# evandez/neuron-descriptions

Hardware: AMD Instinct MI355X
Metric: neuron-descriptions/sec (whole node), 4096 neurons x k=15 exemplars (higher is better)
Workload: dtype f32-equivalent: operands split into (hi,lo) f16 pairs (22 significant bits), 3 f16 MFMAs per product, f32 accumulate

## Files before the change

### include/milan_hip.h

```cpp
#ifndef MILAN_HIP_H
#define MILAN_HIP_H

#include <stddef.h>
#include <stdint.h>

#ifdef __cplusplus
extern "C" {
#endif

#if defined(__GNUC__)
#pragma GCC visibility push(default)
#endif

#define MILAN_ABI_VERSION 11

enum {
  MILAN_OK = 0,
  MILAN_ERR_ARG = -1,
  MILAN_ERR_SHAPE = -2,
  MILAN_ERR_STATE = -3,
  MILAN_ERR_WORKSPACE = -4,
  MILAN_ERR_NO_LM = -5
};

// ... 18 lines not shown
  int32_t embedding_size;
  int32_t attention_size;
  int32_t vocab_size;
  int32_t start_index;
  int32_t stop_index;
  int32_t pad_index;
  int32_t has_lm;
  int32_t lm_hidden_size;
  int32_t lm_embedding_size;
  int32_t lm_layers;
  int32_t trunk_kind;
} milan_dims;

int milan_abi_version(void);
const char* milan_last_error(void);

int milan_create(milan_ctx** out, int device, const milan_dims* dims);
void milan_destroy(milan_ctx* ctx);

int milan_set_weight(milan_ctx* ctx, const char* name, const float* data,
                     const int64_t* shape, int ndim);
int milan_finalize_weights(milan_ctx* ctx, milan_stream stream);

size_t milan_workspace_bytes(const milan_ctx* ctx, int max_neurons, int k,
                             int image_size, int beam_size, int length);

int milan_encode(milan_ctx* ctx, const void* images, int image_dtype,
                 const void* masks, int mask_dtype, int n_images, int height,
                 int width, float* features, void* workspace,
                 size_t workspace_bytes, milan_stream stream);

int milan_encode_spatial(milan_ctx* ctx, const void* images, int image_dtype,
                         const void* masks, int mask_dtype, int n_images,
                         int height, int width, float* out, void* workspace,
                         size_t workspace_bytes, milan_stream stream);

int milan_init_state(milan_ctx* ctx, const float* features, int n, int k,
                     float* h, float* c, void* workspace,
                     size_t workspace_bytes, milan_stream stream);

int milan_step(milan_ctx* ctx, const float* features, int rows, int k,
               const int64_t* tokens, const float* h, const float* c,
               float* h_lm, float* c_lm, float temperature, float* predictions,
               float* attentions, float* h_out, float* c_out, void* workspace,
               size_t workspace_bytes, milan_stream stream);

int milan_decode(milan_ctx* ctx, const float* features, int n, int k,
                 int strategy, int length, int beam_size, int mi,
                 float temperature, int group_size, int64_t* tokens,
                 float* scores, float* predictions, float* attentions,
                 int64_t* beam_tokens, float* beam_scores, int32_t* out_len,
                 void* workspace, size_t workspace_bytes, milan_stream stream);

int milan_lm_score(milan_ctx* ctx, const int64_t* seqs, int rows, int L,
                   const int32_t* seq_len, float* out, void* workspace,
                   size_t workspace_bytes, milan_stream stream);

int milan_lm_logprobs(milan_ctx* ctx, const int64_t* seqs, int rows, int L,
                      float* out, void* workspace, size_t workspace_bytes,
                      milan_stream stream);

int milan_describe(milan_ctx* ctx, const void* images, int image_dtype,
                   const void* masks, int mask_dtype, int n, int k, int height,
                   int width, int strategy, int length, int beam_size, int mi,
                   float temperature, int group_size, float* features_out,
                   int64_t* tokens, float* scores, float* predictions,
                   float* attentions, int64_t* beam_tokens, float* beam_scores,
                   int32_t* out_len, void* workspace, size_t workspace_bytes,
                   milan_stream stream);

int milan_set_graph_capture(milan_ctx* ctx, int enable);
int milan_graph_stats(const milan_ctx* ctx, long long* captures,
                      long long* replays);

enum { MILAN_PRECISION_F32 = 0, MILAN_PRECISION_SPLIT_F16 = 1,
       MILAN_PRECISION_F16 = 2 };

enum { MILAN_FUSE_CHAIN = 1,
       MILAN_FUSE_CHAIN_WIDE = 2,
       MILAN_FUSE_STEM = 4,
       MILAN_FUSE_CONV3 = 8,
       MILAN_FUSE_SKIP_EMPTY = 16,
       MILAN_FUSE_BNECK = 32,
       MILAN_FUSE_SPARSE_TAIL = 64 };
int milan_set_fusion(milan_ctx* ctx, int flags);
int milan_set_precision(milan_ctx* ctx, int precision);
int milan_get_precision(const milan_ctx* ctx);

int milan_set_image_sharing(milan_ctx* ctx, int enable);
int milan_get_image_sharing(const milan_ctx* ctx);
int milan_image_sharing_stats(milan_ctx* ctx, long long* slots,
                              long long* trunk_images, int clear,
                              milan_stream stream);

enum { MILAN_STATUS_SATURATED = 1, MILAN_STATUS_NONFINITE_INPUT = 2 };
int milan_status(milan_ctx* ctx, uint32_t* flags, int clear, milan_stream stream);
int milan_set_act_scale_log2(milan_ctx* ctx, int log2_scale, milan_stream stream);
int milan_get_act_scale_log2(const milan_ctx* ctx);
int milan_encoder_absmax(milan_ctx* ctx, const void* images, int image_dtype,
                         int n_images, int height, int width, float* absmax,
                         void* workspace, size_t workspace_bytes,
                         milan_stream stream);

int milan_profile_enable(int enable);
int milan_profile_read(double* gemm_ms, double* gemm_flops,
                       long long* gemm_launches);

enum milan_stage {
  MILAN_STAGE_OTHER = 0,
  MILAN_STAGE_ENC_INPUT = 1,
  MILAN_STAGE_ENC_STEM = 2,
  MILAN_STAGE_ENC_STEM_TAIL = 3,
  MILAN_STAGE_ENC_LAYER1 = 4,
  MILAN_STAGE_ENC_LAYER2 = 5,
  MILAN_STAGE_ENC_LAYER3 = 6,
  MILAN_STAGE_ENC_LAYER4 = 7,
  MILAN_STAGE_ENC_POOL = 8,
  MILAN_STAGE_DEC_INIT = 9,
  MILAN_STAGE_DEC_SEARCH = 10,
  MILAN_STAGE_DEC_LM = 11,
  MILAN_STAGE_COUNT = 12
};
int milan_profile_read_stages(double* table );

enum milan_kernel_family {
  MILAN_KERNEL_OTHER = 0,
  MILAN_KERNEL_PP32_256 = 1,
  MILAN_KERNEL_PP32_128 = 2,
  MILAN_KERNEL_SPLIT_OTHER = 3,
  MILAN_KERNEL_F32 = 4,
  MILAN_KERNEL_CHAIN = 5,
  MILAN_KERNEL_CHAIN_WIDE = 6,
  MILAN_KERNEL_STEM = 7,
  MILAN_KERNEL_CONV3 = 8,
  MILAN_KERNEL_F16 = 9,
  MILAN_KERNEL_PP32T_256 = 10,
  MILAN_KERNEL_BNECK = 11,
  MILAN_KERNEL_COUNT = 12
};
int milan_profile_read_kernels(double* table );


int milan_exemplar_topk_update(const float* hiddens, int batch, int channels,
                               int hw, const int32_t* units, int n_units,
                               int64_t first_index, int k, int filled,
                               float* pooled_scratch, float* top_values,
                               int64_t* top_index, milan_stream stream);

int milan_exemplar_sketch_append(const float* hiddens, int batch, int channels,
                                 int hw, const int32_t* units, int n_units,
                                 int64_t first, int64_t count, float* level0,
                                 int64_t capacity, int64_t column,
                                 milan_stream stream);

size_t milan_exemplar_sort_workspace(int n_units, int64_t n, int pairs);
int milan_exemplar_sketch_compact(const float* src, int64_t src_capacity,
                                  int64_t n, int n_units, int offset, float* dst,
                                  int64_t dst_capacity, int64_t position,
                                  float* extremes, void* workspace,
                                  size_t workspace_bytes, milan_stream stream);

size_t milan_exemplar_sketch_add_workspace(int n_units, int64_t supplied,
                                           const int64_t* capacities,
                                           int n_levels);
int milan_exemplar_sketch_add(const float* hiddens, int batch, int channels, int hw,
                              const int32_t* units, int n_units, int64_t first,
                              int64_t* consumed, float* const* levels,
// ... 187 lines not shown
```

### neuron-descriptions_amd/csrc/api.hip

```cpp
#include "common.h"

#include <cstdarg>
#include <cstdio>
#include <cstring>

namespace milan {

static thread_local char g_err[1024] = "";

void set_error(const char* fmt, ...) {
  va_list ap;
  va_start(ap, fmt);
  vsnprintf(g_err, sizeof(g_err), fmt, ap);
  va_end(ap);
}

int dev_alloc(milan_ctx* c, void** p, size_t bytes) {
  if (bytes == 0) bytes = 16;
  MILAN_CHECK_HIP(hipMalloc(p, (bytes + 255) & ~size_t(255)));
  c->owned.push_back(*p);
  return 0;
}

__global__ void absmax_kernel(const float* __restrict__ w, long n,
// ... 378 lines not shown

int milan_conv2d_nhwc(const float* x, int n, int h, int w, int cin,
                      const float* weight_oihw, const float* bias, int cout,
                      int kh, int kw, int stride, int pad, int relu,
                      const float* residual, float* y, int precision,
                      milan_stream stream) {
  MILAN_REQUIRE(x && weight_oihw && y, MILAN_ERR_ARG, "conv2d: null argument");
  set_status_word(nullptr);
  const bool force_strip = precision == 3, tap_major = precision == 4, tap_linear = precision == 5;
  if (force_strip || tap_major || tap_linear) precision = MILAN_PRECISION_SPLIT_F16;
  MILAN_REQUIRE(!force_strip || MILAN_EXPERIMENTS, MILAN_ERR_ARG,
                "conv2d: the LDS-strip 3x3 kernel is only in an experiments build "
                "(make EXPERIMENTS=1)");
  MILAN_REQUIRE(precision == MILAN_PRECISION_F32 || cin % 32 == 0,
                MILAN_ERR_SHAPE, "conv2d: split-f16 needs cin %% 32 == 0");
  MILAN_REQUIRE(cin % 4 == 0 && n > 0 && cout > 0, MILAN_ERR_SHAPE,
                "conv2d: cin must be a multiple of 4");
  hipStream_t s = (hipStream_t)stream;
  const int K = kh * kw * cin, Kp = (K + 31) / 32 * 32;
  float *wp = nullptr, *zero = nullptr, *xs = nullptr, *wsp = nullptr, *ws3 = nullptr, *wst = nullptr;
  MILAN_CHECK_HIP(hipMalloc((void**)&wp, sizeof(float) * (size_t)cout * Kp));
  MILAN_CHECK_HIP(hipMalloc((void**)&zero, 256));
  MILAN_CHECK_HIP(hipMemsetAsync(zero, 0, 256, s));
  int r = pack_conv_plain(weight_oihw, cout, cin, kh, kw, wp, s);
  if (r == 0) {
    GemmArgs g{};
    const int ho = (h + 2 * pad - kh) / stride + 1, wo = (w + 2 * pad - kw) / stride + 1;
    g.A = x; g.W = wp; g.bias = bias; g.aux = residual; g.C = y;
    g.M = n * ho * wo; g.N = cout; g.K = K; g.Kp = Kp; g.ldc = cout; g.ldaux = cout;
    g.H = h; g.Wd = w; g.Cin = cin; g.Ho = ho; g.Wo = wo; g.KH = kh; g.KW = kw;
    g.stride = stride; g.pad = pad; g.a_pix_stride = cin;
    g.a_img_stride = (long)h * w * cin;
    g.epilogue = residual ? EPI_BIAS_RES_RELU : (relu ? EPI_BIAS_RELU : EPI_BIAS);
    g.zero = zero;
    if (precision == MILAN_PRECISION_SPLIT_F16) {
      const long rows = (long)n * h * w;
      hipError_t e1 = hipMalloc((void**)&xs, sizeof(float) * (size_t)rows * cin);
      hipError_t e2 = hipMalloc((void**)&wsp, sizeof(float) * (size_t)cout * Kp);
      if (e1 != hipSuccess || e2 != hipSuccess) {
        set_error("conv2d: out of memory");
        r = (int)hipErrorOutOfMemory;
      } else {
        r = launch_f32_to_split(x, cin, xs, cin, rows, cin, 1.f, s);
        if (r == 0)
          r = split_weight_into(wp, cout, Kp, wsp, &g.acc_scale,
                                reinterpret_cast<unsigned int*>(zero) + 32, s);
        g.A = xs; g.W = wsp; g.a_split = 1;
        if (r == 0 && !tap_major && kh * kw > 1 && kh * kw <= 32 && K == Kp) {
          if (hipMalloc((void**)&wst, sizeof(float) * (size_t)cout * Kp) == hipSuccess) {
            r = make_slice_major(wsp, cout, kh * kw, cin, 4, 2, wst, s);
            g.Wt = wst;
            if (tap_linear) g.tap_ncls = -1;
          }
        }
        if (MILAN_EXPERIMENTS && r == 0 && kh == 3 && kw == 3 && stride == 1 &&
            pad == 1 && K == Kp) {
          if (hipMalloc((void**)&ws3, sizeof(float) * (size_t)cout * Kp) == hipSuccess) {
            r = make_chunk_major(wsp, cout, cin, ws3, s);
            g.W3 = ws3;
            if (force_strip) g.tile_hint = 8;
          }
        }
      }
    }
    if (r == 0) r = launch_gemm(g, s);
  }
  hipError_t e = hipStreamSynchronize(s);
  (void)hipFree(wp);
  (void)hipFree(zero);
  if (xs) (void)hipFree(xs);
  if (wsp) (void)hipFree(wsp);
  if (ws3) (void)hipFree(ws3);
  if (wst) (void)hipFree(wst);
  if (r == 0 && e != hipSuccess) {
    set_error("conv2d: %s", hipGetErrorString(e));
    r = (int)e;
  }
  return r;
}

int milan_set_fusion(milan_ctx* c, int flags) {
  MILAN_REQUIRE(c, MILAN_ERR_ARG, "null ctx");
  MILAN_REQUIRE((flags & ~(MILAN_FUSE_CHAIN | MILAN_FUSE_CHAIN_WIDE | MILAN_FUSE_STEM | MILAN_FUSE_CONV3 |
                           MILAN_FUSE_SKIP_EMPTY | MILAN_FUSE_BNECK | MILAN_FUSE_SPARSE_TAIL)) == 0, MILAN_ERR_ARG,
                "unknown fusion flags %d", flags);
  c->fusion = flags;
  return 0;
}

int milan_set_image_sharing(milan_ctx* c, int enable) {
  MILAN_REQUIRE(c, MILAN_ERR_ARG, "null ctx");
  c->share_images = enable != 0;
  return 0;
}

int milan_get_image_sharing(const milan_ctx* c) { return c ? c->share_images : -1; }

int milan_image_sharing_stats(milan_ctx* c, long long* slots, long long* trunk_images, int clear,
                              milan_stream stream) {
  MILAN_REQUIRE(c && slots && trunk_images, MILAN_ERR_ARG,
                "milan_image_sharing_stats: null argument");
  hipStream_t s = (hipStream_t)stream;
  long long host[2] = {0, 0};
  MILAN_CHECK_HIP(hipMemcpyAsync(host, c->share_stats, sizeof(host), hipMemcpyDeviceToHost, s));
  if (clear) MILAN_TRY(launch_zero_fill(c->share_stats, sizeof(host), s));
  MILAN_CHECK_HIP(hipStreamSynchronize(s));
  *slots = host[0];
  *trunk_images = host[1];
  return 0;
}

int milan_set_precision(milan_ctx* c, int precision) {
  MILAN_REQUIRE(c, MILAN_ERR_ARG, "null ctx");
  MILAN_REQUIRE(precision == MILAN_PRECISION_F32 || precision == MILAN_PRECISION_SPLIT_F16 ||
                    precision == MILAN_PRECISION_F16,
                MILAN_ERR_ARG, "unknown precision mode %d", precision);
  c->trunk_f16 = precision == MILAN_PRECISION_F16;
  c->precision = c->trunk_f16 ? MILAN_PRECISION_SPLIT_F16 : precision;
  return 0;
}

int milan_get_precision(const milan_ctx* c) {
  return c ? (c->trunk_f16 ? MILAN_PRECISION_F16 : c->precision) : -1;
}

int milan_profile_enable(int enable) { return gemm_profile_enable(enable); }

int milan_profile_read(double* gemm_ms, double* gemm_flops,
                       long long* gemm_launches) {
  return gemm_profile_read(gemm_ms, gemm_flops, gemm_launches);
}

int milan_profile_read_stages(double* table) {
  MILAN_REQUIRE(table, MILAN_ERR_ARG, "milan_profile_read_stages: null table");
  return profile_read_stages(table);
}

int milan_profile_read_kernels(double* table) {
  MILAN_REQUIRE(table, MILAN_ERR_ARG, "milan_profile_read_kernels: null table");
  return profile_read_kernels(table);
}

int milan_status(milan_ctx* c, uint32_t* flags, int clear, milan_stream stream) {
  MILAN_REQUIRE(c && flags, MILAN_ERR_ARG, "milan_status: null argument");
  hipStream_t s = (hipStream_t)stream;
  unsigned host = 0;
  MILAN_CHECK_HIP(hipMemcpyAsync(&host, c->status, sizeof(host), hipMemcpyDeviceToHost, s));
  if (clear) MILAN_CHECK_HIP(hipMemsetAsync(c->status, 0, sizeof(unsigned), s));
  MILAN_CHECK_HIP(hipStreamSynchronize(s));
  *flags = host;
  return 0;
}

int milan_set_act_scale_log2(milan_ctx* c, int k, milan_stream stream) {
  MILAN_REQUIRE(c, MILAN_ERR_ARG, "null ctx");
  MILAN_REQUIRE(k >= 0 && k <= 10, MILAN_ERR_ARG,
                "activation scale 2^%d outside 2^0 .. 2^10", k);
  MILAN_REQUIRE(c->finalized, MILAN_ERR_STATE, "weights not finalized");
  c->act_scale = ldexpf(1.f, k);
  c->act_scale_log2 = k;
  return encoder_rescale(c, (hipStream_t)stream);
}

int milan_get_act_scale_log2(const milan_ctx* c) { return c ? c->act_scale_log2 : -1; }

int milan_encoder_absmax(milan_ctx* c, const void* images, int image_dtype, int n_images,
                         int height, int width, float* absmax, void* workspace,
                         size_t workspace_bytes, milan_stream stream) {
// ... 62 lines not shown
```

### neuron-descriptions_amd/csrc/common.h

```cpp
#pragma once
#include <hip/hip_runtime.h>
#include <stdint.h>
#include <stddef.h>
#include <string>
#include <vector>
#include <map>

#include "../../include/milan_hip.h"

#ifndef MILAN_EXPERIMENTS
#define MILAN_EXPERIMENTS 0
#endif

namespace milan {

void set_error(const char* fmt, ...);
#define MILAN_CHECK_HIP(expr)                                              \
  do {                                                                     \
    hipError_t _e = (expr);                                                \
    if (_e != hipSuccess) {                                                \
      milan::set_error("%s:%d: %s -> %s", __FILE__, __LINE__, #expr,       \
                       hipGetErrorString(_e));                             \
      return (int)_e;                                                      \
    }                                                                      \
  } while (0)
#define MILAN_REQUIRE(cond, code, ...)                                     \
  do {                                                                     \
    if (!(cond)) {                                                         \
      milan::set_error(__VA_ARGS__);                                       \
      return (code);                                                       \
    }                                                                      \
  } while (0)
#define MILAN_TRY(expr)                                                    \
  do {                                                                     \
    int _r = (expr);                                                       \
    if (_r != 0) return _r;                                                \
  } while (0)

enum Epilogue : int {
  EPI_BIAS = 0,
  EPI_BIAS_RELU = 1,
  EPI_BIAS_RES_RELU = 2,
  EPI_BIAS_TANH = 3,
  EPI_BIAS_SIGMUL = 4,
  EPI_BIAS_ADD = 5,
  EPI_LSTM = 6,
  EPI_LSE = 7,
};

constexpr int MILAN_TAP_CLASSES = 9;
struct GemmArgs {
  const float* A;
  const float* W;
  const float* bias;
  const float* aux;
  float* C;
  int M, N, K, Kp;
  int ldc, ldaux;
  int H, Wd, Cin, Ho, Wo, KH, KW, stride, pad;
  long a_pix_stride;
  long a_img_stride;
  int epilogue;
  const float* zero;
  int flop_k;
  int a_split;
  int out_split;
  int aux_split;
  float acc_scale;
  int out_mode;
  const float* W3;
  const float* A2;
  int K1, H2, W2d, stride2;
  long a2_pix_stride, a2_img_stride;
  int aniso, stride_w, pad_w;
  int debug;
  int tile_hint;
  int stagger;
  long long* prof;
  int chunk_major;
  float* C2;
  float* Cs;
  unsigned* status;
  int f16;
  const float* Wt;
  int tap_inner;
  const long long* lse_tgt;
  long lse_tgt_stride;
  float* lse_x;
  const int* m_live;
  int m_live_mul;
  int tap_ncls;
  int tap_cls[MILAN_TAP_CLASSES][5];
};
static_assert(sizeof(GemmArgs) % 4 == 0, "GemmArgs is reloaded word by word");

enum OutMode : int { OUT_SCALAR = 0, OUT_VEC4 = 1, OUT_SPLIT8 = 2, OUT_F16 = 3 };

int launch_gemm(const GemmArgs& g, hipStream_t s);
void set_status_word(unsigned* word);
unsigned* status_word();
void profile_tag_kernel(int family);
int launch_zero_fill(void* p, size_t bytes, hipStream_t s);
int launch_f32_to_split(const float* src, long ld_src, float* dst, long ld_dst,
                        long rows, int K, float scale, hipStream_t s);
int gemm_profile_enable(int enable);
int ensure_lds_attr(const void* kern, int bytes);
int device_cus8(int* out);
void* gemm_profile_begin(double flops, double bytes, hipStream_t s);
void gemm_profile_end(void* rec, hipStream_t s);

struct ShareArgs {
  const unsigned char* images;
  long bytes;
  int n;
  int hash_bits;
  int skip_empty;
  const int* list_n;
  const int* bbox;
  void* hash;
  int *rep, *flag;
  int *order, *bbox_c, *count, *class_of;
};
int launch_image_classes(const ShareArgs& a, hipStream_t s);
int launch_share_count(long long* stats, int n, const int* live, hipStream_t s);

struct ChainArgs {
  const float* T2;
  const float* W3;
  const float* bias3;
  const float* R;
  float* X;
  const float* W1;
  const float* bias1;
  float* T1;
  int M, P;
  const float* A2;
  int KD;
  float scale3, scale1;
  long long* prof;
  int NR;
  unsigned* status;
  const int* m_live;
  int m_live_mul;
  const float* C2in;
  const float* W2;
  const float* bias2;
  float scale2;
  int ch, cw;
  const float* W0;
  const float* bias0;
  float scale0;
};
bool chain_supported(int P, int KD, int NR = 0);
bool chain_conv_supported(int P, int KD, int NR, int h, int w);
bool chain_conv_c1_supported(int P, int KD, int NR, int h, int w);
int launch_chain(const ChainArgs& a, hipStream_t s);
struct StemArgs {
  const float* in;
  const float* ws;
  const float* bias;
  float acc_scale;
  const float* scale;
  const float* shift;
  float* raw;
  float* y;
  const int* bbox;
  const float* zero;
  int n, H, G, h1, w1, hp, wp;
  int tiles_y, tiles_x;
  int debug;
  unsigned* status;
  const unsigned char* in_u8;
  const unsigned* lut;
  const int* order;
  int W;
  const int* n_live;
};
bool stem_fused_supported(int cout, int Kp);
int launch_stem_fused(const StemArgs& a, hipStream_t s);
struct Conv3Args {
  const float* in;
// ... 119 lines not shown

__device__ __forceinline__ float cvt_pk_f16(float a, float b) {
  float r;
  asm("v_cvt_pk_f16_f32 %0, %1, %2" : "=v"(r) : "v"(a), "v"(b));
  return r;
}
template <int SEL>
__device__ __forceinline__ float mix_sub_f16(float x, float hpair) {
  float r;
  if constexpr (SEL == 0)
    asm("v_fma_mix_f32 %0, -%1, 1.0, %2 op_sel:[0,0,0] op_sel_hi:[1,0,0]" : "=v"(r) : "v"(hpair), "v"(x));
  else
    asm("v_fma_mix_f32 %0, -%1, 1.0, %2 op_sel:[1,0,0] op_sel_hi:[1,0,0]" : "=v"(r) : "v"(hpair), "v"(x));
  return r;
}
template <int SEL>
__device__ __forceinline__ float mix_add_f16(float hpair, float lpair) {
  float r;
  if constexpr (SEL == 0)
    asm("v_fma_mix_f32 %0, %1, 1.0, %2 op_sel:[0,0,0] op_sel_hi:[1,0,1]" : "=v"(r) : "v"(hpair), "v"(lpair));
  else
    asm("v_fma_mix_f32 %0, %1, 1.0, %2 op_sel:[1,0,1] op_sel_hi:[1,0,1]" : "=v"(r) : "v"(hpair), "v"(lpair));
  return r;
}
__device__ __forceinline__ float max3_abs(float a, float b, float c) {
  float r;
  asm("v_max3_f32 %0, |%1|, |%2|, |%3|" : "=v"(r) : "v"(a), "v"(b), "v"(c));
  return r;
}
__device__ __forceinline__ float sat_fold8(const float* x, float sat) {
  return max3_abs(max3_abs(x[0], x[1], x[2]), max3_abs(x[3], x[4], x[5]), max3_abs(x[6], x[7], sat));
}
__device__ __forceinline__ void report_saturation(unsigned* status, float sat) {
  if (status != nullptr && sat >= 65504.f) atomicOr(status, 1u );
}
template <typename V4>
__device__ __forceinline__ void split8_rne(const float* v, V4* hi_out, V4* lo_out, float* sat = nullptr) {
  V4 hi, lo;
  float x[8];
#pragma unroll
  for (int d = 0; d < 4; ++d) {
    asm("v_med3_f32 %0, %1, %2, %3" : "=v"(x[2 * d]) : "v"(v[2 * d]), "v"(-65504.f), "v"(65504.f));
    asm("v_med3_f32 %0, %1, %2, %3" : "=v"(x[2 * d + 1]) : "v"(v[2 * d + 1]), "v"(-65504.f), "v"(65504.f));
    hi[d] = cvt_pk_f16(x[2 * d], x[2 * d + 1]);
    lo[d] = cvt_pk_f16(mix_sub_f16<0>(x[2 * d], hi[d]), mix_sub_f16<1>(x[2 * d + 1], hi[d]));
  }
  if (sat) *sat = sat_fold8(x, *sat);
  *hi_out = hi;
  *lo_out = lo;
}
template <typename V4>
__device__ __forceinline__ void split8_relu_rne(const float* v, V4* hi_out, V4* lo_out, float* sat = nullptr) {
  V4 hi, lo;
  float x[8];
#pragma unroll
  for (int d = 0; d < 4; ++d) {
    asm("v_med3_f32 %0, %1, 0, %2" : "=v"(x[2 * d]) : "v"(v[2 * d]), "v"(65504.f));
    asm("v_med3_f32 %0, %1, 0, %2" : "=v"(x[2 * d + 1]) : "v"(v[2 * d + 1]), "v"(65504.f));
    hi[d] = cvt_pk_f16(x[2 * d], x[2 * d + 1]);
    lo[d] = cvt_pk_f16(mix_sub_f16<0>(x[2 * d], hi[d]), mix_sub_f16<1>(x[2 * d + 1], hi[d]));
  }
  if (sat) *sat = sat_fold8(x, *sat);
  *hi_out = hi;
  *lo_out = lo;
}
template <typename V4>
__device__ __forceinline__ void join8_exact(V4 hi, V4 lo, float* v) {
#pragma unroll
  for (int d = 0; d < 4; ++d) {
    v[2 * d] = mix_add_f16<0>(hi[d], lo[d]);
    v[2 * d + 1] = mix_add_f16<1>(hi[d], lo[d]);
  }
}

}

struct milan_ctx {
  int device = 0;
  milan_dims d{};
  bool finalized = false;
  int precision = 0;
  int trunk_f16 = 0;
  int fusion = MILAN_FUSE_CHAIN | MILAN_FUSE_CHAIN_WIDE | MILAN_FUSE_STEM | MILAN_FUSE_CONV3 |
               MILAN_FUSE_SKIP_EMPTY | MILAN_FUSE_BNECK | MILAN_FUSE_SPARSE_TAIL;
  int graph_capture = 0;
  struct GraphEntry { std::vector<char> key; hipGraphExec_t exec = nullptr; int seen = 0; };
  std::vector<GraphEntry> graphs;
  long graph_replays = 0, graph_captures = 0;
  float* scratch = nullptr;
  size_t scratch_floats = 0;
  std::map<std::string, milan::Tensor> raw;
  std::vector<void*> owned;
  float* zero = nullptr;
  milan::ConvW stem;
  milan::ConvW stem_pair;
  milan::ConvW alex[5];
  float *bn1_scale = nullptr, *bn1_shift = nullptr;
  float act_scale = 32.f;
  int act_scale_log2 = 5;
  float *bn1_scale_s = nullptr, *bn1_shift_s = nullptr;
  unsigned* stem_lut = nullptr;
  unsigned* status = nullptr;
  unsigned* calib = nullptr;
  int share_images = 0;
  int share_hash_bits = 64;
  long long* share_stats = nullptr;
  std::vector<milan::Bottleneck> blocks[4];
  float mean[3] = {0.485f, 0.456f, 0.406f}, stdv[3] = {0.229f, 0.224f, 0.225f};
  milan::LinearW init_h, init_c, q2h, k2h, gate, lstm_ih, lstm_hh, out;
  milan::LinearW lstm_cat;
  float *att_w = nullptr, *att_b = nullptr;
  float* embedding = nullptr;
  std::vector<milan::LinearW> lm_ih, lm_hh;
  std::vector<milan::LinearW> lm_cat;
  milan::LinearW lm_out;
  float* lm_embedding = nullptr;
};

namespace milan {
int dev_alloc(milan_ctx* c, void** p, size_t bytes);
int make_split_weight(milan_ctx* c, const float* w, int n, int kp, float** ws,
                      float* ws_inv, hipStream_t s);
int pack_conv_plain(const float* w_oihw, int cout, int cin, int kh, int kw,
                    float* wp, hipStream_t s);
int encoder_finalize(milan_ctx* c, hipStream_t s);
int encoder_rescale(milan_ctx* c, hipStream_t s);
int make_slice_major(const float* ws, int cout, int taps, int cin, int gps, int gb, float* dst,
                     hipStream_t s);
int make_chunk_major(const float* ws, int cout, int cin, float* dst,
                     hipStream_t s);
size_t encoder_workspace(const milan_ctx* c, int n_images, int H, int W);
int encoder_run_spatial(milan_ctx* c, const void* images, int image_dtype,
                        const void* masks, int mask_dtype, int n, int H, int W,
                        float* out, milan::Arena& ws, hipStream_t s);
int encoder_run(milan_ctx* c, const void* images, int image_dtype,
                const void* masks, int mask_dtype, int n_images, int H, int W,
                float* features, Arena& ws, hipStream_t s);
int decoder_finalize(milan_ctx* c, hipStream_t s);
size_t decoder_workspace(const milan_ctx* c, int n, int k, int beam, int length);
int decoder_init_state(milan_ctx* c, const float* features, int n, int k,
                       float* h, float* cc, Arena& ws, hipStream_t s);
int decoder_step(milan_ctx* c, const float* features, int rows, int k,
                 const int64_t* tokens, const float* h, const float* cc,
                 float* h_lm, float* c_lm, float temperature,
                 float* predictions, float* attentions, float* h_out,
                 float* c_out, Arena& ws, hipStream_t s);
int decoder_decode(milan_ctx* c, const float* features, int n, int k,
                   int strategy, int length, int beam, int mi,
                   float temperature, int group_size, int64_t* tokens,
                   float* scores, float* predictions, float* attentions,
                   int64_t* beam_tokens, float* beam_scores, int32_t* out_len,
                   Arena& ws, hipStream_t s);
int decoder_lm_logprobs(milan_ctx* c, const int64_t* seqs, int rows, int L,
                        float* out, milan::Arena& ws, hipStream_t s);
int decoder_lm_score(milan_ctx* c, const int64_t* seqs, int rows, int L,
                     const int32_t* seq_len, float* out, Arena& ws,
                     hipStream_t s);
}
```

### neuron-descriptions_amd/csrc/encoder.hip

```cpp
#include "common.h"
#include <optional>
#include <vector>

#include <cstdlib>

namespace milan {

static constexpr float kBnEps = 1e-5f;

__global__ void pack_conv_kernel(const float* __restrict__ w, int cout, int cin,
                                 int cinp, int kh, int kw, int kp,
                                 const float* __restrict__ gamma,
                                 const float* __restrict__ beta,
                                 const float* __restrict__ mean,
                                 const float* __restrict__ var,
                                 float* __restrict__ wp,
                                 float* __restrict__ bias) {
  const long total = (long)cout * kp;
  for (long idx = blockIdx.x * (long)blockDim.x + threadIdx.x; idx < total;
       idx += (long)gridDim.x * blockDim.x) {
    const int o = idx / kp, k = idx - (long)o * kp;
    const int tap = k / cinp, i = k - tap * cinp;
    float v = 0.f;
    if (tap < kh * kw && i < cin) {
// ... 769 lines not shown
  if constexpr (SHARED) {
    img = blockIdx.x;
    const int cls = class_of[img];
    if (cls < img0 || cls >= img0 + ncls) return;
    trow = cls - img0;
  } else {
    const int slot_img = blockIdx.x + img0;
    if (live != nullptr && slot_img >= *live) return;
    img = order ? order[slot_img] : slot_img;
    trow = blockIdx.x;
  }
  const int lane = threadIdx.x & 63, wave = threadIdx.x >> 6;
  const int G = C / 8, pw = 64 / lpp;
  const int gl = lane % lpp, sub = lane / lpp;
  const int g = blockIdx.y * 64 + gl;
  const int slot = wave * pw + sub, nslots = 4 * pw;
  const long base = (long)img * lv.per_image + lv.off[level];
  const int cnt = list_n[img * 5 + level];
  const float* t = tap + (long)trow * P * C + (long)g * 8;
  float a0[8], a1[8];
#pragma unroll
  for (int e = 0; e < 8; ++e) { a0[e] = 0.f; a1[e] = 0.f; }
  auto add = [&](int i, float (&acc)[8]) {
    const float* q = t + (long)list_idx[base + i] * C;
    const float w = list_w[base + i];
    const f32x4_t hi = *reinterpret_cast<const f32x4_t*>(q);
    const f32x4_t lo = *reinterpret_cast<const f32x4_t*>(q + 4);
    float v[8];
    join8_exact(hi, lo, v);
#pragma unroll
    for (int e = 0; e < 8; ++e) acc[e] += w * v[e];
  };
  if (g < G) {
    int i = slot;
    for (; i + nslots < cnt; i += 2 * nslots) { add(i, a0); add(i + nslots, a1); }
    if (i < cnt) add(i, a0);
  }
#pragma unroll
  for (int e = 0; e < 8; ++e) part[(wave * 64 + lane) * 8 + e] = a0[e] + a1[e];
  __syncthreads();
  if (wave == 0 && sub == 0 && g < G) {
    float sum[8];
#pragma unroll
    for (int e = 0; e < 8; ++e) sum[e] = 0.f;
    for (int w = 0; w < 4; ++w)
      for (int sb = 0; sb < pw; ++sb)
#pragma unroll
        for (int e = 0; e < 8; ++e) sum[e] += part[(w * 64 + sb * lpp + gl) * 8 + e];
    const bool bad = poison != nullptr && poison[img];
    float* f = features + (long)img * fstride + col_off + g * 8;
#pragma unroll
    for (int e = 0; e < 8; ++e) f[e] = bad ? __builtin_nanf("") : sum[e] * inv_scale;
  }
}

__global__ void poison_fill_kernel(float* __restrict__ out, long per_image, int n,
                                   const int* __restrict__ poison) {
  const long total = (long)n * per_image;
  for (long i = blockIdx.x * (long)blockDim.x + threadIdx.x; i < total;
       i += (long)gridDim.x * blockDim.x)
    if (poison[i / per_image]) out[i] = __builtin_nanf("");
}

__global__ void act_absmax_kernel(const float* __restrict__ x, long n,
                                  unsigned* __restrict__ out) {
  float m = 0.f;
  for (long i = blockIdx.x * (long)blockDim.x + threadIdx.x; i < n;
       i += (long)gridDim.x * blockDim.x) {
    const float a = fabsf(x[i]);
    m = (a > m || a != a) ? a : m;
  }
  for (int o = 32; o > 0; o >>= 1) {
    const float t = __shfl_xor(m, o);
    m = (t > m || t != t) ? t : m;
  }
  if ((threadIdx.x & 63) == 0) atomicMax(out, __float_as_uint(m));
}


constexpr int kTailMaxP = 1024;

__global__ __launch_bounds__(64) void tail_union_kernel(
    const int* __restrict__ list_idx, const int* __restrict__ list_n, Levels lv,
    const int* __restrict__ class_of, int P, unsigned char* __restrict__ s0) {
  const int i = blockIdx.x, c = class_of[i];
  if (c < 0) return;
  const long base = (long)i * lv.per_image + lv.off[4];
  const int cnt = list_n[i * 5 + 4];
  for (int e = threadIdx.x; e < cnt; e += 64) s0[(long)c * P + list_idx[base + e]] = 1;
}

__global__ __launch_bounds__(64) void tail_sets_kernel(
    const int* __restrict__ list_idx, const int* __restrict__ list_n, Levels lv,
    const int* __restrict__ order, const int* __restrict__ live, int n,
    int* __restrict__ loc, int* __restrict__ cnt,
    const unsigned char* __restrict__ s0 = nullptr) {
  __shared__ unsigned char s[3][kTailMaxP];
  const int j = blockIdx.x, lane = threadIdx.x;
  const int h = lv.h[4], w = lv.w[4], P = h * w;
  if (live != nullptr && j >= *live) {
    if (lane < 3) cnt[lane * n + j] = 0;
    return;
  }
  const int img = order ? order[j] : j;
  if (s0 != nullptr) {
    for (int p = lane; p < P; p += 64) s[0][p] = s0[(long)j * P + p];
  } else {
    for (int p = lane; p < P; p += 64) s[0][p] = 0;
    __syncthreads();
    const long base = (long)img * lv.per_image + lv.off[4];
    const int c = list_n[img * 5 + 4];
    for (int i = lane; i < c; i += 64) s[0][list_idx[base + i]] = 1;
  }
  __syncthreads();
  for (int k = 1; k < 3; ++k) {
    for (int p = lane; p < P; p += 64) {
      const int y = p / w, x = p - y * w;
      unsigned char v = 0;
      for (int dy = -1; dy <= 1; ++dy)
        for (int dx = -1; dx <= 1; ++dx) {
          const int yy = y + dy, xx = x + dx;
          if (yy >= 0 && yy < h && xx >= 0 && xx < w) v |= s[k - 1][yy * w + xx];
        }
      s[k][p] = v;
    }
    __syncthreads();
  }
  for (int k = 0; k < 3; ++k) {
    int count = 0;
    int* out = loc + ((long)k * n + j) * P;
    for (int p0 = 0; p0 < P; p0 += 64) {
      const int p = p0 + lane;
      const bool nz = p < P && s[k][p];
      const unsigned long long m = __ballot(nz);
      if (nz) out[count + __popcll(m & ((1ull << lane) - 1ull))] = p;
      count += __popcll(m);
    }
    if (lane == 0) cnt[k * n + j] = count;
  }
}

__global__ __launch_bounds__(256) void tail_scan_kernel(const int* __restrict__ cnt, int n,
                                                        int* __restrict__ off, int* __restrict__ U) {
  __shared__ int tmp[256];
  const int k = blockIdx.x, tid = threadIdx.x;
  int base = 0;
  for (int j0 = 0; j0 < n; j0 += 256) {
    const int j = j0 + tid;
    const int v = j < n ? cnt[(long)k * n + j] : 0;
    tmp[tid] = v;
    __syncthreads();
    for (int o = 1; o < 256; o <<= 1) {
      const int add = tid >= o ? tmp[tid - o] : 0;
      __syncthreads();
      tmp[tid] += add;
      __syncthreads();
    }
    if (j < n) off[(long)k * n + j] = base + tmp[tid] - v;
    base += tmp[255];
    __syncthreads();
  }
  if (tid == 0) U[k] = base;
}

__global__ void tail_fill_kernel(const int* __restrict__ loc, const int* __restrict__ cnt,
                                 const int* __restrict__ off, int n, int P, int* __restrict__ rows) {
  const int j = blockIdx.x, k = blockIdx.y;
  const int c = cnt[k * n + j], o = off[k * n + j];
  for (int i = threadIdx.x; i < c; i += blockDim.x)
    rows[(long)k * n * P + o + i] = j * P + loc[((long)k * n + j) * P + i];
}

template <bool SCATTER>
__global__ void tail_rows_kernel(const float4* __restrict__ src, const int* __restrict__ idx,
                                 const int* __restrict__ live, int w4, float4* __restrict__ dst) {
  const long total = (long)*live * w4;
  for (long i = blockIdx.x * (long)blockDim.x + threadIdx.x; i < total;
       i += (long)gridDim.x * blockDim.x) {
    const long u = i / w4;
    const int q = (int)(i - u * w4);
    if (SCATTER) dst[(long)idx[u] * w4 + q] = src[i];
    else dst[i] = src[(long)idx[u] * w4 + q];
  }
}

__global__ void tail_im2col_kernel(const float4* __restrict__ t1, const int* __restrict__ rows,
                                   const int* __restrict__ live, int h, int w, int C,
                                   float4* __restrict__ acol) {
  const int per = 9 * C / 4, P = h * w, c4 = C / 4;
  const long total = (long)*live * per;
  for (long i = blockIdx.x * (long)blockDim.x + threadIdx.x; i < total;
       i += (long)gridDim.x * blockDim.x) {
    const long u = i / per;
    const int q = (int)(i - u * per);
    const int sl = q / 72, r = q - sl * 72, tap = r >> 3, f = r & 7;
    const int row = rows[u];
    const int j = row / P, p = row - j * P;
    const int y = p / w + tap / 3 - 1, x = p % w + tap % 3 - 1;
    float4 v = make_float4(0.f, 0.f, 0.f, 0.f);
    if (y >= 0 && y < h && x >= 0 && x < w)
      v = t1[((long)j * P + y * w + x) * c4 + sl * 8 + f];
    acol[i] = v;
  }
}

struct EncPlan {
  Levels lv;
  int h1, w1, hp, wp;
  float *in4, *raw, *x0, *x1, *ds, *t1, *t2;
  size_t x_sz, t1_sz, t2_sz;
  int *list_idx, *list_n;
  float* list_w;
  int* bbox;
  int* poison;
  int *order, *bbox_c, *count;
  int *tail_loc, *tail_cnt, *tail_off, *tail_rows, *tail_U;
  void* sh_hash;
  int *sh_rep, *sh_flag, *class_of;
  unsigned char* tail_s0;
};

static int conv_out(int h, int k, int s, int p) { return (h + 2 * p - k) / s + 1; }

static int plan(const milan_ctx* c, int n, int H, int W, Arena& a, EncPlan* pl) {
  const int wd = c->d.trunk_width;
  pl->h1 = conv_out(H, 7, 2, 3); pl->w1 = conv_out(W, 7, 2, 3);
  pl->hp = conv_out(pl->h1, 3, 2, 1); pl->wp = conv_out(pl->w1, 3, 2, 1);
  Levels& lv = pl->lv;
  lv.h[0] = pl->h1; lv.w[0] = pl->w1;
  lv.h[1] = pl->hp; lv.w[1] = pl->wp;
  for (int l = 2; l < 5; ++l) {
    lv.h[l] = conv_out(lv.h[l - 1], 3, 2, 1);
    lv.w[l] = conv_out(lv.w[l - 1], 3, 2, 1);
  }
  long off = 0;
  for (int l = 0; l < 5; ++l) { lv.off[l] = off; off += (long)lv.h[l] * lv.w[l]; }
  lv.per_image = off;
  const int exp = c->d.trunk_kind == MILAN_TRUNK_BASIC ? 1 : 4;
  size_t x_sz = (size_t)pl->hp * pl->wp * wd, t1_sz = 0, t2_sz = 0;
  for (int li = 0; li < 4; ++li) {
    const size_t planes = (size_t)wd << li;
    const size_t in_px = (size_t)lv.h[li == 0 ? 1 : li] * lv.w[li == 0 ? 1 : li];
    const size_t out_px = (size_t)lv.h[li + 1] * lv.w[li + 1];
    x_sz = x_sz > out_px * planes * exp ? x_sz : out_px * planes * exp;
    t1_sz = t1_sz > in_px * planes ? t1_sz : in_px * planes;
    t2_sz = t2_sz > out_px * planes ? t2_sz : out_px * planes;
  }
  pl->x_sz = x_sz; pl->t1_sz = t1_sz; pl->t2_sz = t2_sz;
  pl->in4 = a.get<float>((size_t)n * H * (W + 2) * 4);
  pl->raw = a.get<float>((size_t)n * pl->h1 * pl->w1 * wd);
  pl->x0 = a.get<float>((size_t)n * x_sz);
  pl->x1 = a.get<float>((size_t)n * x_sz);
  pl->ds = a.get<float>((size_t)n * x_sz);
  pl->t1 = a.get<float>((size_t)n * t1_sz);
  pl->t2 = a.get<float>((size_t)n * t2_sz);
  pl->list_idx = a.get<int>((size_t)n * lv.per_image);
  pl->list_w = a.get<float>((size_t)n * lv.per_image);
  pl->list_n = a.get<int>((size_t)n * 5);
  pl->bbox = a.get<int>((size_t)n * 4);
  pl->poison = a.get<int>((size_t)n);
  pl->order = a.get<int>((size_t)n);
  pl->bbox_c = a.get<int>((size_t)n * 4);
  pl->count = a.get<int>(4);
  {
    const size_t P4 = (size_t)lv.h[4] * lv.w[4];
    pl->tail_loc = a.get<int>(3 * (size_t)n * P4);
    pl->tail_rows = a.get<int>(3 * (size_t)n * P4);
    pl->tail_cnt = a.get<int>(3 * (size_t)n);
    pl->tail_off = a.get<int>(3 * (size_t)n);
    pl->tail_U = a.get<int>(4);
    pl->sh_hash = a.get<unsigned long long>((size_t)n);
    pl->sh_rep = a.get<int>((size_t)n);
    pl->sh_flag = a.get<int>((size_t)n);
    pl->class_of = a.get<int>((size_t)n);
    pl->tail_s0 = a.get<unsigned char>(((size_t)n * P4 + 3) & ~(size_t)3);
  }
  return 0;
}

static int encoder_sub_batch() {
  static int v = 0;
  if (v == 0) {
    const char* e = getenv("MILAN_ENC_SUB");
    v = e ? atoi(e) : 9600;
    if (v < 1) v = 9600;
  }
  return v;
}

static void alexnet_workspace_dry(const milan_ctx* c, int n, int H, int W,
                                  Arena& a);

size_t encoder_workspace(const milan_ctx* c, int n_images, int H, int W) {
  Arena a; a.dry = true;
  const int sub = encoder_sub_batch();
  const int n = n_images < sub ? n_images : sub;
  if (c->d.trunk_kind == MILAN_TRUNK_NONE) return 0;
  if (c->d.trunk_kind == MILAN_TRUNK_ALEXNET) {
    alexnet_workspace_dry(c, n, H, W, a);
    return a.off;
  }
  EncPlan pl;
  plan(c, n, H, W, a, &pl);
  return a.off;
}

static GemmArgs conv_args(const ConvW& cw, const float* in, int n, int H, int W,
                          float* out, int epi, const float* aux,
                          const float* zero, int* Ho, int* Wo,
                          bool split = false, bool scaled_bias = true) {
  GemmArgs g{};
  *Ho = conv_out(H, cw.kh, cw.stride, cw.pad);
  *Wo = conv_out(W, cw.kw, cw.stride, cw.pad);
  g.A = in; g.W = cw.w; g.bias = cw.bias; g.aux = aux; g.C = out;
  g.M = n * (*Ho) * (*Wo); g.N = cw.cout; g.K = cw.K; g.Kp = cw.Kp;
  g.ldc = cw.cout; g.ldaux = cw.cout;
  g.H = H; g.Wd = W; g.Cin = cw.cin; g.Ho = *Ho; g.Wo = *Wo;
  g.KH = cw.kh; g.KW = cw.kw; g.stride = cw.stride; g.pad = cw.pad;
  g.a_pix_stride = cw.cin;
  g.a_img_stride = (long)H * W * cw.cin;
  g.epilogue = epi; g.zero = zero;
  g.flop_k = cw.kh * cw.kw * cw.cin_real;
  if (split) {
    g.W = cw.ws; g.a_split = 1; g.out_split = 1; g.aux_split = aux != nullptr;
    g.acc_scale = cw.ws_inv;
    g.W3 = cw.ws3;
    g.Wt = cw.wst;
    if (scaled_bias && cw.bias_s) g.bias = cw.bias_s;
  }
  return g;
}

static GemmArgs conv_args_f16(const ConvW& cw, const float* in, int n, int H, int W,
                              float* out, int epi, const float* aux, const float* zero,
                              int* Ho, int* Wo) {
  GemmArgs g = conv_args(cw, in, n, H, W, out, epi, aux, zero, Ho, Wo, true);
  g.W = cw.wf; g.W3 = nullptr; g.Wt = cw.wft;
  g.f16 = 1; g.out_split = 0; g.aux_split = 0;
  g.Cin = cw.cin / 2; g.K = cw.K / 2; g.Kp = cw.Kp / 2;
  g.a_pix_stride = cw.cin / 2;
  g.a_img_stride = (long)H * W * (cw.cin / 2);
  g.ldc = cw.cout / 2; g.ldaux = cw.cout / 2;
  return g;
}

static int encoder_run_batch(milan_ctx* c, const void* images, int image_dtype,
                             const void* masks, int mask_dtype, int n, int H,
                             int W, float* features, Arena& ws, hipStream_t s,
                             float* spatial_out = nullptr);
static int alexnet_run_batch(milan_ctx* c, const void* images, int image_dtype,
                             const void* masks, int mask_dtype, int n, int H,
                             int W, float* features, Arena& ws, hipStream_t s);

int encoder_run(milan_ctx* c, const void* images, int image_dtype,
                const void* masks, int mask_dtype, int n, int H, int W,
                float* features, Arena& ws, hipStream_t s) {
  const int sub = encoder_sub_batch();
  const size_t isz = image_dtype == MILAN_DTYPE_U8 ? 1 : 4;
// ... 227 lines not shown
    else
      hipLaunchKernelGGL(masked_pool_kernel<0>, dim3(cnt, (C + 63) / 64),
                         dim3(256), 0, s, tap, P, C, level, pl.lv, pl.list_idx,
                         pl.list_w, pl.list_n, features, F, col_off, img0, 1.f, poison, order, live);
    MILAN_CHECK_HIP(hipGetLastError());
    return 0;
  };

  int ho, wo;
  {
    GemmArgs g = conv_args(c->stem, pl.in4, n, H, W, pl.raw, EPI_BIAS, nullptr,
                           c->zero, &ho, &wo);
    if (pair_stem) {
      g = conv_args(c->stem_pair, pl.in4, n, H, G, pl.raw, EPI_BIAS, nullptr,
                    c->zero, &ho, &wo, true);
      g.Ho = ho = pl.h1; g.Wo = wo = pl.w1;
      g.M = n * ho * wo;
      g.aniso = 1; g.stride_w = 1; g.pad_w = 1;
      g.out_split = 0;
      g.flop_k = c->stem.kh * c->stem.kw * c->stem.cin_real;
    }
    const bool fused_stem = pair_stem && (c->fusion & MILAN_FUSE_STEM) &&
                            stem_fused_supported(c->stem_pair.cout, c->stem_pair.Kp);
    if (fused_stem) {
      StemArgs sa{};
      sa.in = pl.in4; sa.ws = c->stem_pair.ws; sa.bias = c->stem_pair.bias;
      if (stem_u8) {
        sa.in = nullptr; sa.in_u8 = (const unsigned char*)images; sa.lut = c->stem_lut;
        sa.order = order; sa.W = W;
      }
      sa.n_live = live;
      sa.acc_scale = c->stem_pair.ws_inv;
      sa.scale = c->bn1_scale_s; sa.shift = c->bn1_shift_s;
      sa.raw = spatial ? nullptr : pl.raw; sa.y = pl.x0;
      sa.bbox = spatial ? nullptr : bbox;
      sa.zero = c->zero;
      sa.n = n; sa.H = H; sa.G = G; sa.h1 = pl.h1; sa.w1 = pl.w1;
      sa.hp = pl.hp; sa.wp = pl.wp;
      {
        StageScope scope(MILAN_STAGE_ENC_STEM, s);
        MILAN_TRY(launch_stem_fused(sa, s));
      }
      MILAN_TRY(pool(pl.raw, 0, wd, 0));
    } else {
    {
      StageScope scope(MILAN_STAGE_ENC_STEM, s);
      MILAN_TRY(launch_live(g));
    }
    MILAN_TRY(pool(pl.raw, 0, wd, 0));
    stage.emplace(MILAN_STAGE_ENC_STEM_TAIL, s);
    const long total = (long)n * pl.hp * pl.wp * (wd / (split ? 8 : 4));
    const int blocks = (int)((total + 255) / 256 < 16384 ? (total + 255) / 256 : 16384);
    if (split)
      hipLaunchKernelGGL(bn_relu_maxpool_split_kernel, dim3(blocks), dim3(256), 0,
                         s, pl.raw, n, pl.h1, pl.w1, wd, pl.hp, pl.wp,
                         c->bn1_scale_s, c->bn1_shift_s, pl.x0, c->status, live);
    else
      hipLaunchKernelGGL(bn_relu_maxpool_kernel, dim3(blocks), dim3(256), 0, s,
                         (const float4*)pl.raw, n, pl.h1, pl.w1, wd / 4, pl.hp,
                         pl.wp, (const float4*)c->bn1_scale,
                         (const float4*)c->bn1_shift, (float4*)pl.x0, live);
    MILAN_CHECK_HIP(hipGetLastError());
    stage.reset();
    }
    if (c->calib && !split) {
      MILAN_TRY(track(pl.x0, (long)n * pl.hp * pl.wp * wd));
    }
  }

  auto gemm_t = [&](const GemmArgs& g) -> int {
    MILAN_TRY(launch_live(g));
    if (c->calib && !split) MILAN_TRY(track(g.C, (long)g.M * g.N));
    return 0;
  };
  const int P4 = pl.lv.h[4] * pl.lv.w[4];
  bool tail = split && !fast && !spatial && masks != nullptr && c->calib == nullptr &&
              (c->fusion & MILAN_FUSE_SPARSE_TAIL) && c->d.trunk_kind == MILAN_TRUNK_BOTTLENECK &&
              c->blocks[3].size() >= 2 && P4 >= 1 && P4 <= kTailMaxP;
  if (tail) {
    const Bottleneck& lb = c->blocks[3].back();
    const size_t need = (size_t)P4 * ((size_t)2 * lb.c1.cin + lb.c3.cout + (size_t)11 * lb.c1.cout);
    tail = need <= (size_t)pl.h1 * pl.w1 * wd;
  }
  if (tail) {
    const unsigned char* s0 = nullptr;
    if (class_of != nullptr) {
      MILAN_TRY(launch_zero_fill(pl.tail_s0, ((size_t)n * P4 + 3) & ~(size_t)3, s));
      hipLaunchKernelGGL(tail_union_kernel, dim3(n), dim3(64), 0, s, pl.list_idx, pl.list_n, pl.lv,
                         class_of, P4, pl.tail_s0);
      s0 = pl.tail_s0;
    }
    hipLaunchKernelGGL(tail_sets_kernel, dim3(n), dim3(64), 0, s, pl.list_idx, pl.list_n, pl.lv,
                       order, live, n, pl.tail_loc, pl.tail_cnt, s0);
    hipLaunchKernelGGL(tail_scan_kernel, dim3(3), dim3(256), 0, s, pl.tail_cnt, n, pl.tail_off,
                       pl.tail_U);
    hipLaunchKernelGGL(tail_fill_kernel, dim3(n, 3), dim3(64), 0, s, pl.tail_loc, pl.tail_cnt,
                       pl.tail_off, n, P4, pl.tail_rows);
    MILAN_CHECK_HIP(hipGetLastError());
  }
  auto tail_block_ok = [&](const Bottleneck& b) {
    return !b.basic && !b.has_down && b.c1.ws && b.c2.ws && b.c2.wst && b.c3.ws && b.c1.bias_s &&
           b.c2.bias_s && b.c3.bias_s && b.c1.kh == 1 && b.c1.kw == 1 && b.c1.stride == 1 &&
           b.c2.kh == 3 && b.c2.kw == 3 && b.c2.stride == 1 && b.c2.pad == 1 && b.c3.kh == 1 &&
           b.c3.kw == 1 && b.c3.stride == 1 && b.c1.K == b.c1.Kp && b.c2.K == b.c2.Kp &&
           b.c3.K == b.c3.Kp && b.c1.cout % 32 == 0 && b.c2.cin == b.c1.cout &&
           b.c2.cout == b.c1.cout && b.c3.cin == b.c1.cout && b.c3.cout == b.c1.cin &&
           b.c1.cin % 4 == 0;
  };
  auto tail_block = [&](const Bottleneck& b, const float* X, float* Y, float* T1, int hh,
                        int ww, int kM, int kO) -> int {
    const long rows_all = (long)n * P4;
    const int Cin = b.c1.cin, P = b.c1.cout, Cout = b.c3.cout;
    float* xg = pl.raw;
    float* t1c = xg + rows_all * Cin;
    float* acol = t1c + rows_all * P;
    float* t2c = acol + rows_all * 9 * P;
    float* rg = t2c + rows_all * P;
    float* yc = rg + rows_all * Cin;
    const int* rowsM = pl.tail_rows + (long)kM * n * P4;
    const int* rowsO = pl.tail_rows + (long)kO * n * P4;
    const int* UM = pl.tail_U + kM;
    const int* UO = pl.tail_U + kO;
    auto blocks_for = [](long items) { return (int)((items + 255) / 256 < 8192 ? (items + 255) / 256 : 8192); };
    auto lin = [&](const float* A, int K, const ConvW& cw, const float* W, float* C, int N, int epi,
                   const float* aux, const int* U) -> int {
      GemmArgs g = linear_args(A, K, W, cw.bias_s, C, N, (int)rows_all, N, K, epi, c->zero, aux, N);
      g.a_split = 1; g.out_split = 1; g.aux_split = aux != nullptr;
      g.acc_scale = cw.ws_inv;
      g.flop_k = cw.kh * cw.kw * cw.cin_real;
      g.m_live = U; g.m_live_mul = 1;
      return launch_gemm(g, s);
    };
    hipLaunchKernelGGL(tail_rows_kernel<false>, dim3(blocks_for(rows_all * (Cin / 4))), dim3(256), 0, s,
                       (const float4*)X, rowsM, UM, Cin / 4, (float4*)xg);
    MILAN_TRY(lin(xg, Cin, b.c1, b.c1.ws, t1c, P, EPI_BIAS_RELU, nullptr, UM));
    hipLaunchKernelGGL(tail_rows_kernel<true>, dim3(blocks_for(rows_all * (P / 4))), dim3(256), 0, s,
                       (const float4*)t1c, rowsM, UM, P / 4, (float4*)T1);
    hipLaunchKernelGGL(tail_im2col_kernel, dim3(blocks_for(rows_all * (9 * P / 4))), dim3(256), 0, s,
                       (const float4*)T1, rowsO, UO, hh, ww, P, (float4*)acol);
    MILAN_TRY(lin(acol, 9 * P, b.c2, b.c2.wst, t2c, P, EPI_BIAS_RELU, nullptr, UO));
    hipLaunchKernelGGL(tail_rows_kernel<false>, dim3(blocks_for(rows_all * (Cin / 4))), dim3(256), 0, s,
                       (const float4*)X, rowsO, UO, Cin / 4, (float4*)rg);
    MILAN_TRY(lin(t2c, P, b.c3, b.c3.ws, yc, Cout, EPI_BIAS_RES_RELU, rg, UO));
    hipLaunchKernelGGL(tail_rows_kernel<true>, dim3(blocks_for(rows_all * (Cout / 4))), dim3(256), 0, s,
                       (const float4*)yc, rowsO, UO, Cout / 4, (float4*)Y);
    MILAN_CHECK_HIP(hipGetLastError());
    return 0;
  };

  float *x = pl.x0, *y = pl.x1;
  int h = pl.hp, w = pl.wp, col = wd;
  bool t1_ready = false;
  float *t1buf = pl.t1, *t1alt = pl.ds;
  for (int li = 0; li < 4; ++li) {
    stage.emplace(MILAN_STAGE_ENC_LAYER1 + li, s);
    const std::vector<Bottleneck>& blocks = c->blocks[li];
    if (fast && li == 2) {
      const long groups = (long)n * h * w * ((wd * 4) << 1) / 8;
      const int nb = (int)((groups + 255) / 256 < 16384 ? (groups + 255) / 256 : 16384);
      hipLaunchKernelGGL(split_to_f16_kernel, dim3(nb), dim3(256), 0, s, x, groups, pl.ds, live,
                         groups / n);
      MILAN_CHECK_HIP(hipGetLastError());
      y = x; x = pl.ds;
    }
    for (size_t bi = 0; bi < blocks.size(); ++bi) {
      const Bottleneck& b = blocks[bi];
      int h1, w1, h2, w2, h3, w3;
      if (fast && li >= 2) {
        GemmArgs g1 = conv_args_f16(b.c1, x, n, h, w, pl.t1, EPI_BIAS_RELU, nullptr, c->zero, &h1, &w1);
        MILAN_TRY(launch_live(g1));
        GemmArgs g2 = conv_args_f16(b.c2, pl.t1, n, h1, w1, pl.t2, EPI_BIAS_RELU, nullptr, c->zero, &h2, &w2);
        MILAN_TRY(launch_live(g2));
        if (b.has_down) {
          GemmArgs g3 = conv_args_f16(b.c3d, pl.t2, n, h2, w2, y, EPI_BIAS_RELU, nullptr, c->zero, &h3, &w3);
          g3.Cin = b.c3.cin / 2;
          g3.a_pix_stride = b.c3.cin / 2;
          g3.a_img_stride = (long)h2 * w2 * (b.c3.cin / 2);
          g3.A2 = x; g3.K1 = b.c3.K / 2; g3.H2 = h; g3.W2d = w;
          g3.stride2 = b.down.stride;
          g3.a2_pix_stride = b.down.cin / 2;
          g3.a2_img_stride = (long)h * w * (b.down.cin / 2);
          g3.flop_k = b.c3.K + b.down.K;
          MILAN_TRY(launch_live(g3));
        } else {
          GemmArgs g3 = conv_args_f16(b.c3, pl.t2, n, h2, w2, y, EPI_BIAS_RES_RELU, x, c->zero, &h3, &w3);
          MILAN_TRY(launch_live(g3));
        }
        float* tmp = x; x = y; y = tmp;
        h = h3; w = w3;
        continue;
      }
      if (tail && li == 3 && bi >= 1 && bi + 2 >= blocks.size() && tail_block_ok(b) &&
          (bi + 1 == blocks.size() || tail_block_ok(blocks.back())) &&
          h == pl.lv.h[4] && w == pl.lv.w[4]) {
        const int kO = bi + 1 == blocks.size() ? 0 : 1;
        MILAN_TRY(tail_block(b, x, y, t1buf, h, w, kO + 1, kO));
        float* tmp = x; x = y; y = tmp;
        continue;
      }
      if (b.basic) {
        GemmArgs g1 = conv_args(b.c1, x, n, h, w, pl.t1, EPI_BIAS_RELU, nullptr,
                                c->zero, &h1, &w1, split);
        MILAN_TRY(gemm_t(g1));
        const float* identity = x;
        if (b.has_down) {
          int hd, wdn;
          GemmArgs gd = conv_args(b.down, x, n, h, w, pl.ds, EPI_BIAS, nullptr,
                                  c->zero, &hd, &wdn, split);
          MILAN_TRY(gemm_t(gd));
          identity = pl.ds;
        }
        GemmArgs g2 = conv_args(b.c2, pl.t1, n, h1, w1, y, EPI_BIAS_RES_RELU,
                                identity, c->zero, &h3, &w3, split);
        MILAN_TRY(gemm_t(g2));
        float* tmp = x; x = y; y = tmp;
        h = h3; w = w3;
        continue;
      }
      GemmArgs g1 = conv_args(b.c1, x, n, h, w, t1buf, EPI_BIAS_RELU, nullptr,
                              c->zero, &h1, &w1, split);
      const bool c1_pending = !t1_ready;
      t1_ready = false;
      GemmArgs g2 = conv_args(b.c2, t1buf, n, h1, w1, pl.t2, EPI_BIAS_RELU,
                              nullptr, c->zero, &h2, &w2, split);
#if MILAN_EXPERIMENTS
      {
        static const bool taps_inner = getenv("MILAN_TAPS_INNER") && atoi(getenv("MILAN_TAPS_INNER"));
        if (split && taps_inner && b.c2.ws3 && b.c2.cin >= 128 && b.c2.cout > 64) {
          g2.W = b.c2.ws3;
          g2.chunk_major = 1;
          g2.W3 = nullptr;
        }
      }
#endif
      const bool last_of_stage = bi + 1 == blocks.size();
      const Bottleneck* nbp = !last_of_stage ? &blocks[bi + 1]
                              : (li + 1 < 4 && !c->blocks[li + 1].empty())
                                    ? &c->blocks[li + 1][0] : nullptr;
      bool chain_plain = false, chain_ds = false;
      int chain_P = 0, chain_NR = 0;
      if (split && nbp != nullptr && !(fast && last_of_stage && li + 1 >= 2) && !b.basic &&
          (c->fusion & (b.c3.cin >= 256 ? MILAN_FUSE_CHAIN_WIDE : MILAN_FUSE_CHAIN))) {
        const Bottleneck& nb = *nbp;
        chain_P = b.c3.cin;
        chain_NR = last_of_stage ? 2 * chain_P : chain_P;
        const bool shapes = !nb.basic && nb.has_down == last_of_stage && nb.c1.ws &&
                            b.c3.ws && b.c3.kh == 1 && b.c3.kw == 1 && b.c3.stride == 1 &&
                            b.c3.K == b.c3.Kp && b.c3.cout == 4 * chain_P &&
                            nb.c1.kh == 1 && nb.c1.kw == 1 && nb.c1.stride == 1 &&
                            nb.c1.cin == 4 * chain_P && nb.c1.cout == chain_NR &&
                            nb.c1.K == nb.c1.Kp && b.c3.bias && nb.c1.bias;
        h2 = conv_out(h1, b.c2.kh, b.c2.stride, b.c2.pad);
        w2 = conv_out(w1, b.c2.kw, b.c2.stride, b.c2.pad);
        chain_plain = shapes && !b.has_down && chain_supported(chain_P, 0, chain_NR);
        chain_ds = shapes && b.has_down && b.c3d.ws && b.down.kh == 1 &&
                   b.down.kw == 1 && b.down.stride == 1 && h2 == h &&
                   w2 == w && chain_supported(chain_P, b.down.cin, chain_NR);
      }
      const bool conv_front =
          (chain_plain || chain_ds) && (c->fusion & MILAN_FUSE_BNECK) && b.c2.K == b.c2.Kp &&
          b.c2.bias_s && conv3_p64_supported(b.c2.cin, b.c2.cout, b.c2.kh, b.c2.kw, b.c2.stride,
                                             b.c2.pad) &&
          chain_conv_supported(chain_P, chain_ds ? b.down.cin : 0, chain_NR, h1, w1);
      const bool c1_front =
          conv_front && c1_pending && chain_ds && b.c1.ws && b.c1.bias_s && b.c1.kh == 1 &&
          b.c1.kw == 1 && b.c1.stride == 1 && b.c1.cin == 64 && b.c1.cout == 64 &&
          b.c1.K == b.c1.Kp && h1 == h && w1 == w &&
          chain_conv_c1_supported(chain_P, b.down.cin, chain_NR, h1, w1);
      if (c1_pending && !c1_front) MILAN_TRY(gemm_t(g1));
      if (conv_front) {
      } else if (split && (c->fusion & MILAN_FUSE_CONV3) && b.c2.K == b.c2.Kp &&
          conv3_p64_supported(b.c2.cin, b.c2.cout, b.c2.kh, b.c2.kw, b.c2.stride,
                              b.c2.pad)) {
        Conv3Args ca{};
        ca.in = t1buf; ca.ws = b.c2.ws; ca.bias = b.c2.bias_s; ca.acc_scale = b.c2.ws_inv;
        ca.out = pl.t2; ca.zero = c->zero; ca.n = n; ca.h = h1; ca.w = w1;
        ca.n_live = live;
        MILAN_TRY(launch_conv3_p64(ca, s));
      } else {
        MILAN_TRY(gemm_t(g2));
      }
      const float* identity = x;
      if (chain_plain || chain_ds) {
        const Bottleneck& nb = *nbp;
        ChainArgs ca{};
        ca.T2 = pl.t2; ca.X = y; ca.W1 = nb.c1.ws; ca.bias1 = nb.c1.bias_s;
        ca.T1 = t1buf; ca.M = n * h2 * w2; ca.P = chain_P; ca.scale1 = nb.c1.ws_inv;
        ca.NR = chain_NR;
        ca.m_live = live; ca.m_live_mul = h2 * w2;
        if (conv_front) {
          ca.C2in = t1buf; ca.W2 = b.c2.ws; ca.bias2 = b.c2.bias_s; ca.scale2 = b.c2.ws_inv;
          ca.ch = h1; ca.cw = w1;
          ca.T2 = nullptr; ca.T1 = t1alt;
          if (c1_front) {
            ca.C2in = x; ca.W0 = b.c1.ws; ca.bias0 = b.c1.bias_s; ca.scale0 = b.c1.ws_inv;
          }
        }
        if (chain_plain) {
          ca.W3 = b.c3.ws; ca.bias3 = b.c3.bias_s; ca.R = x; ca.scale3 = b.c3.ws_inv;
        } else {
          ca.W3 = b.c3d.ws; ca.bias3 = b.c3d.bias_s; ca.A2 = x; ca.KD = b.down.cin;
          ca.scale3 = b.c3d.ws_inv;
        }
        MILAN_TRY(launch_chain(ca, s));
        if (conv_front) { float* tt = t1buf; t1buf = t1alt; t1alt = tt; }
        t1_ready = true;
        float* tmp = x; x = y; y = tmp;
        h = h2; w = w2;
        continue;
      }
      if (b.has_down && split && b.c3d.ws && b.c3d.cout > 64) {
        int h3, w3;
        GemmArgs g3 = conv_args(b.c3d, pl.t2, n, h2, w2, y, EPI_BIAS_RELU,
                                nullptr, c->zero, &h3, &w3, true);
        g3.Cin = b.c3.cin;
        g3.a_pix_stride = b.c3.cin;
        g3.a_img_stride = (long)h2 * w2 * b.c3.cin;
        g3.A2 = x; g3.K1 = b.c3.K; g3.H2 = h; g3.W2d = w;
        g3.stride2 = b.down.stride;
        g3.a2_pix_stride = b.down.cin;
        g3.a2_img_stride = (long)h * w * b.down.cin;
        g3.flop_k = b.c3.K + b.down.K;
        MILAN_TRY(gemm_t(g3));
        float* tmp = x; x = y; y = tmp;
        h = h3; w = w3;
        continue;
      }
      if (b.has_down) {
        int hd, wdn;
        GemmArgs gd = conv_args(b.down, x, n, h, w, pl.ds, EPI_BIAS, nullptr,
                                c->zero, &hd, &wdn, split);
        MILAN_TRY(gemm_t(gd));
        identity = pl.ds;
      }
      GemmArgs g3 = conv_args(b.c3, pl.t2, n, h2, w2, y, EPI_BIAS_RES_RELU,
                              identity, c->zero, &h3, &w3, split);
      MILAN_TRY(gemm_t(g3));
      float* tmp = x; x = y; y = tmp;
      h = h3; w = w3;
    }
    stage.reset();
    const int C = (c->d.trunk_kind == MILAN_TRUNK_BASIC ? wd : wd * 4) << li;
    MILAN_REQUIRE(h == pl.lv.h[li + 1] && w == pl.lv.w[li + 1], MILAN_ERR_SHAPE,
                  "internal: stage %d geometry mismatch", li + 1);
    MILAN_TRY(pool(x, li + 1, C, col));
    col += C;
  }
  if (spatial) {
    const int C = (c->d.trunk_kind == MILAN_TRUNK_BASIC ? wd : wd * 4) << 3;
    const long rows = (long)n * h * w;
    if (split) {
      const long total = rows * (C / 8);
      const int blocks = (int)((total + 255) / 256 < 16384 ? (total + 255) / 256 : 16384);
      hipLaunchKernelGGL(split_to_f32_kernel, dim3(blocks), dim3(256), 0, s, x,
                         total, spatial_out, 1.f / c->act_scale);
      MILAN_CHECK_HIP(hipGetLastError());
    } else {
      MILAN_CHECK_HIP(hipMemcpyAsync(spatial_out, x, sizeof(float) * rows * C,
                                     hipMemcpyDeviceToDevice, s));
    }
    if (poison) {
      const long per_image = (long)h * w * C;
      const long total = (long)n * per_image;
      const int blocks = (int)((total + 255) / 256 < 4096 ? (total + 255) / 256 : 4096);
      hipLaunchKernelGGL(poison_fill_kernel, dim3(blocks), dim3(256), 0, s, spatial_out,
                         per_image, n, poison);
      MILAN_CHECK_HIP(hipGetLastError());
    }
  }
  return 0;
}

int encoder_rescale(milan_ctx* c, hipStream_t s) {
  auto redo = [&](const float* src, float* dst, int n) -> int {
    if (!src || !dst) return 0;
    hipLaunchKernelGGL(scale_vec_kernel, dim3((n + 255) / 256), dim3(256), 0, s, src,
                       c->act_scale, n, dst);
    MILAN_CHECK_HIP(hipGetLastError());
    return 0;
  };
  if (c->stem.w) {
    MILAN_TRY(redo(c->bn1_scale, c->bn1_scale_s, c->stem.cout));
    MILAN_TRY(redo(c->bn1_shift, c->bn1_shift_s, c->stem.cout));
  }
  for (int li = 0; li < 4; ++li)
    for (Bottleneck& b : c->blocks[li])
      for (ConvW* w : {&b.c1, &b.c2, &b.c3, &b.down, &b.c3d})
        MILAN_TRY(redo(w->bias, w->bias_s, w->cout));
  return 0;
}


__global__ void maxpool3s2_f32_kernel(const float4* __restrict__ x, int n, int H,
                                      int W, int C4, int Ho, int Wo, int pad,
                                      float4* __restrict__ y) {
  const long total = (long)n * Ho * Wo * C4;
  for (long idx = blockIdx.x * (long)blockDim.x + threadIdx.x; idx < total;
       idx += (long)gridDim.x * blockDim.x) {
    const int cc = idx % C4;
    long t = idx / C4;
    const int wo = t % Wo; t /= Wo;
    const int ho = t % Ho;
    const long img = t / Ho;
    float4 best = make_float4(-INFINITY, -INFINITY, -INFINITY, -INFINITY);
    for (int dy = 0; dy < 3; ++dy) {
// ... 204 lines not shown
```

### neuron-descriptions_amd/csrc/gemm.hip

```cpp
#include "common.h"

#include <map>
#include <mutex>
#include <utility>

#include <cstdio>
#include <cstdlib>
#include <cstring>
#include <type_traits>
#include <utility>
#include <vector>

#ifndef MILAN_ABLATE_BUILD
#define MILAN_ABLATE_BUILD 0
#endif
#ifndef MILAN_EXPERIMENTS
#define MILAN_EXPERIMENTS 0
#endif

namespace milan {

typedef float f32x16 __attribute__((ext_vector_type(16)));
typedef float f32x4 __attribute__((ext_vector_type(4)));
typedef _Float16 f16x8 __attribute__((ext_vector_type(8)));
// ... 1117 lines not shown
        for (int it = 0; it < B_ITERS; ++it) issue_b(it, kt_issue, nxt_slot);
        __builtin_amdgcn_sched_barrier(0);
      }
#pragma unroll
      for (int i = 0; i < TM; ++i) {
        if (i + 1 < TM) {
          ah[i + 1] = *reinterpret_cast<const f32x4*>(Ab + aoff[i + 1] +
                                                      ((chi ^ aswz[i + 1]) << 2));
          al[i + 1] = *reinterpret_cast<const f32x4*>(Ab + aoff[i + 1] +
                                                      ((clo ^ aswz[i + 1]) << 2));
        }
        if constexpr (STEADY) {
          if constexpr (DMA_POS == 0) {
            if (i < A_ITERS) issue_a(ra, i, kt_issue, nxt_slot);
            else issue_b(i - A_ITERS, kt_issue, nxt_slot);
          }
        } else {
          if (i < A_ITERS && has_next) issue_a(ra_n, i, kt_issue, nxt_slot);
        }
#pragma unroll
        for (int j = 0; j < TN; ++j) {
          acc[i][j] = __builtin_amdgcn_mfma_f32_32x32x16_f16(
              as_f16x8(ah[i]), as_f16x8(bl[j]), acc[i][j], 0, 0, 0);
          acc[i][j] = __builtin_amdgcn_mfma_f32_32x32x16_f16(
              as_f16x8(al[i]), as_f16x8(bh[j]), acc[i][j], 0, 0, 0);
          acc[i][j] = __builtin_amdgcn_mfma_f32_32x32x16_f16(
              as_f16x8(ah[i]), as_f16x8(bh[j]), acc[i][j], 0, 0, 0);
        }
      }
      if constexpr (STEADY && DMA_POS == 2) {
        __builtin_amdgcn_sched_barrier(0);
#pragma unroll
        for (int it = 0; it < A_ITERS; ++it) issue_a(ra, it, kt_issue, nxt_slot);
#pragma unroll
        for (int it = 0; it < B_ITERS; ++it) issue_b(it, kt_issue, nxt_slot);
      }
    };
    auto advance = [&]() { cur = cur + 1 == STAGES ? 0 : cur + 1; };
    auto slot_ahead = [&]() { const int n = cur + AHEAD; return n >= STAGES ? n - STAGES : n; };

    auto steady_loop = [&](auto pos_tag) {
      for (int kt = 0; kt + AHEAD < nk; ++kt) {
        compute(cur, slot_ahead(), kt + AHEAD, std::true_type{}, pos_tag);
        asm volatile("s_waitcnt vmcnt(%0)" ::"n"((AHEAD - 1) * LOADS) : "memory");
        __builtin_amdgcn_s_barrier();
        advance();
      }
    };
    if (wave < NT_WAVES / 2) steady_loop(std::integral_constant<int, 1>{});
    else steady_loop(std::integral_constant<int, 2>{});
#pragma unroll
    for (int t = 0; t < AHEAD; ++t) {
      compute(cur, slot_ahead(), t, std::false_type{}, std::integral_constant<int, 0>{});
      if (t + 1 < AHEAD) {
        if (has_next) {
          if (t == 0) asm volatile("s_waitcnt vmcnt(%0)" ::"n"(2 * LOADS + A_ITERS) : "memory");
          else if (t == 1) asm volatile("s_waitcnt vmcnt(%0)" ::"n"(LOADS + 2 * A_ITERS) : "memory");
          else asm volatile("s_waitcnt vmcnt(%0)" ::"n"(3 * A_ITERS) : "memory");
        } else {
          if (t == 0) asm volatile("s_waitcnt vmcnt(%0)" ::"n"(2 * LOADS) : "memory");
          else if (t == 1) asm volatile("s_waitcnt vmcnt(%0)" ::"n"(LOADS) : "memory");
          else asm volatile("s_waitcnt vmcnt(0)" ::: "memory");
        }
        __builtin_amdgcn_s_barrier();
      }
      advance();
    }
    __builtin_amdgcn_s_barrier();
#pragma unroll
    for (int i = 0; i < TM; ++i)
#pragma unroll
      for (int j = 0; j < TN; ++j) acc[i][j] = acc[i][j] * g.acc_scale;
    run_epilogue<TM, TN>(g, acc, Bs, wave, lane, tile_m * BM + wm * WROWS,
                         tile_n * BN + wn * 64);
    if (!has_next) break;
    __builtin_amdgcn_s_barrier();
    q += gridDim.x;
    tile_m = ntile_m; tile_n = ntile_n;
#pragma unroll
    for (int it = 0; it < A_ITERS; ++it) ra[it] = ra_n[it];
  }
}

__device__ __forceinline__ GemmArgs reload_gemm_args() {
  typedef const int __attribute__((address_space(4)))* KArgWords;
  KArgWords kw = (KArgWords)__builtin_amdgcn_kernarg_segment_ptr();
  asm volatile("" : "+s"(kw));
  GemmArgs g;
  int words[sizeof(GemmArgs) / 4];
#pragma unroll
  for (unsigned i = 0; i < sizeof(GemmArgs) / 4; ++i) words[i] = kw[i];
  __builtin_memcpy(&g, words, sizeof(GemmArgs));
  g.M = live_rows(g.m_live, g.m_live_mul, g.M);
  return g;
}


__device__ __forceinline__ void split16_pp_tile(int tile_m, int tile_n, int tid) {
  const GemmArgs g = reload_gemm_args();
  constexpr int BM = 256, BN = 256, BK = 16, S = 4, TM = 4, TN = 2, LOADS = 4;
  constexpr unsigned OOB = 0x80000000u;
  extern __shared__ __attribute__((aligned(16))) float smem[];
  float* As = smem;
  float* Bs = smem + S * BM * BK;
  const int lane = tid & 63;
  const int wave = __builtin_amdgcn_readfirstlane(tid >> 6);
  const int wm = wave >> 2, wn = wave & 3;

  const int lrow = tid >> 2;
  const int kc = (tid & 3) ^ ((tid >> 4) & 3);
  const int HoWo = g.Ho * g.Wo;
  const int img0 = (tile_m * BM) / HoWo;
  const long bias = ((long)g.pad * g.Wd + g.pad) * g.a_pix_stride;
  const __amdgpu_buffer_rsrc_t srd_a = __builtin_amdgcn_make_buffer_rsrc(
      const_cast<float*>(g.A + (long)img0 * g.a_img_stride - bias), 0, 0x7fffffff, 0x00020000);
  const __amdgpu_buffer_rsrc_t srd_a2 = __builtin_amdgcn_make_buffer_rsrc(
      const_cast<float*>(g.A2 ? g.A2 + (long)img0 * g.a2_img_stride : g.A), 0, 0x7fffffff,
      0x00020000);
  const __amdgpu_buffer_rsrc_t srd_w = __builtin_amdgcn_make_buffer_rsrc(
      const_cast<float*>(g.W + (long)tile_n * BN * g.Kp), 0, 0x7fffffff, 0x00020000);
  unsigned row_off[2], row_off2[2], voff[2], vb[2];
  int hi0[2], wi0[2];
#pragma unroll
  for (int it = 0; it < 2; ++it) {
    const int m = tile_m * BM + it * 128 + lrow;
    const bool ok = m < g.M;
    const int mm = ok ? m : g.M - 1;
    const int img = mm / HoWo;
    const int rem = mm - img * HoWo;
    const int ho = rem / g.Wo, wo = rem - ho * g.Wo;
    hi0[it] = ho * g.stride - g.pad;
    wi0[it] = wo * g.stride - g.pad;
    row_off[it] = ok ? (unsigned)(((long)(img - img0) * g.a_img_stride +
                                   ((long)hi0[it] * g.Wd + wi0[it]) * g.a_pix_stride + bias +
                                   kc * 4) * 4)
                     : OOB;
    row_off2[it] = (ok && g.A2)
                       ? (unsigned)(((long)(img - img0) * g.a2_img_stride +
                                     ((long)(ho * g.stride2) * g.W2d + wo * g.stride2) *
                                         g.a2_pix_stride + kc * 4) * 4)
                       : OOB;
    const int n = tile_n * BN + it * 128 + lrow;
    vb[it] = n < g.N ? (unsigned)(((long)(it * 128 + lrow) * g.Kp + kc * 4) * 4) : OOB;
  }
  const int nk = g.Kp / BK;
  const int k1_tiles = g.A2 ? g.K1 / BK : 0x7fffffff;
  int is_kt = 0, is_kh = 0, is_kw = 0, is_cin0 = 0, seg_soff = 0;
  int cin_limit = g.Cin;
  __amdgpu_buffer_rsrc_t cur_srd = srd_a;
  auto set_tap = [&]() {
#pragma unroll
    for (int it = 0; it < 2; ++it) {
      const bool inb = (unsigned)(hi0[it] + is_kh) < (unsigned)g.H &&
                       (unsigned)(wi0[it] + is_kw) < (unsigned)g.Wd;
      voff[it] = inb ? row_off[it] : OOB;
    }
    seg_soff = (int)((((long)is_kh * g.Wd + is_kw) * g.a_pix_stride) * 4);
  };
  set_tap();
  auto issue_tile = [&](auto slot_tag) {
    constexpr int SLOT = decltype(slot_tag)::value;
    int woff = wave * (16 * BK);
    asm volatile("" : "+s"(woff));
    float* adst = As + SLOT * (BM * BK) + woff;
    float* bdst = Bs + SLOT * (BN * BK) + woff;
    const int soff = seg_soff + is_cin0 * 4;
    __builtin_amdgcn_raw_ptr_buffer_load_lds(cur_srd, (LDS_AS void*)adst, 16, voff[0], soff, 0, 0);
    __builtin_amdgcn_raw_ptr_buffer_load_lds(cur_srd, (LDS_AS void*)(adst + 128 * BK), 16, voff[1],
                                             soff, 0, 0);
    const int woffk = is_kt * (BK * 4);
    __builtin_amdgcn_raw_ptr_buffer_load_lds(srd_w, (LDS_AS void*)bdst, 16, vb[0], woffk, 0, 0);
    __builtin_amdgcn_raw_ptr_buffer_load_lds(srd_w, (LDS_AS void*)(bdst + 128 * BK), 16, vb[1],
                                             woffk, 0, 0);
    if (is_kt + 1 < nk) {
      ++is_kt;
      is_cin0 += BK;
// ... 103 lines not shown
  } else {
    phase_barrier();
    auto step = [&](auto slot_tag) {
      read_phase(slot_tag);
      asm volatile("s_waitcnt vmcnt(%0)" ::"n"((S - 2) * LOADS) : "memory");
      phase_barrier();
      multiply();
      phase_barrier();
    };
    int kt = 0;
    for (; kt + 4 <= nk; kt += 4) {
      step(std::integral_constant<int, 0>{});
      step(std::integral_constant<int, 1>{});
      step(std::integral_constant<int, 2>{});
      step(std::integral_constant<int, 3>{});
    }
    if (kt < nk) {
      step(std::integral_constant<int, 0>{});
      step(std::integral_constant<int, 1>{});
    }
  }
  asm volatile("s_waitcnt vmcnt(0)" ::: "memory");
  __builtin_amdgcn_s_barrier();
  const GemmArgs ge = reload_gemm_args();
#pragma unroll
  for (int i = 0; i < TM; ++i)
#pragma unroll
    for (int j = 0; j < TN; ++j) acc[i][j] = acc[i][j] * ge.acc_scale;
  run_epilogue<TM, TN>(ge, acc, smem, wave, lane, tile_m * BM + wm * 128, tile_n * BN + wn * 64);
}

struct PpLoader {
  __amdgpu_buffer_rsrc_t srd_a, srd_a2, srd_w, cur_srd;
  unsigned row_off[4], row_off2[4], voff[4], vb[4];
  int hw0[4];
  unsigned mask[4];
  int ia, iw, is_kh, is_kw, is_cin0, seg_soff, cin_limit;
  unsigned a_bits, w_bits;
  int w_slice;
};

struct TapTile {
  int y0, ny, x0, nx;
  unsigned mask;
  int cnt, j, tile_n;
};

__device__ __forceinline__ bool tap_tile(const GemmArgs& g, int tiles_m, int tiles_n, TapTile* t) {
  const int b = blockIdx.x;
  if (g.tap_ncls == 0) {
    const int T = tiles_m * tiles_n;
    if (b >= T) return false;
    const int tile = xcd_tile(b, T);
    t->j = tile / tiles_n;
    t->tile_n = tile - t->j * tiles_n;
    t->y0 = 0; t->ny = g.Ho; t->x0 = 0; t->nx = g.Wo;
    t->mask = 0xffffffffu >> (32 - g.KH * g.KW);
    t->cnt = g.M;
    return true;
  }
  typedef const int __attribute__((address_space(4)))* KArgWords;
  const KArgWords cw = (KArgWords)__builtin_amdgcn_kernarg_segment_ptr() + offsetof(GemmArgs, tap_cls) / 4;
  const int imgs = g.M / (g.Ho * g.Wo);
  int first = 0, cls = -1, cfirst = 0, ctiles = 0;
#pragma unroll
  for (int c = 0; c < MILAN_TAP_CLASSES; ++c) {
    const int T = c < g.tap_ncls ? ((imgs * cw[c * 5 + 1] * cw[c * 5 + 3] + 255) >> 8) * tiles_n : 0;
    const int B = (T + 7) & ~7;
    if (cls < 0 && b < first + B) { cls = c; cfirst = first; ctiles = T; }
    first += B;
  }
  if (cls < 0) return false;
  const int bl = b - cfirst;
  if ((bl >> 3) >= (ctiles >> 3) + ((bl & 7) < (ctiles & 7))) return false;
  const int tile = xcd_tile(bl, ctiles);
  t->j = tile / tiles_n;
  t->tile_n = tile - t->j * tiles_n;
  t->y0 = cw[cls * 5]; t->ny = cw[cls * 5 + 1]; t->x0 = cw[cls * 5 + 2]; t->nx = cw[cls * 5 + 3];
  t->mask = (unsigned)cw[cls * 5 + 4];
  t->cnt = imgs * t->ny * t->nx;
  return true;
}

template <int BNW, bool F16 = false, bool TAPI = false>
__device__ __forceinline__ void split16_pp32_tile(int tile_m, int tile_n, int tid, bool prefetched,
                                                  bool has_next, int ntile_m, int ntile_n,
                                                  TapTile tt = TapTile{}) {
  const GemmArgs g = reload_gemm_args();
  constexpr int BM = 256, BN = 256, BKP = 32, TM = BNW == 256 ? 4 : 2, TN = 2;
  static_assert(BNW == 256 || BNW == 128, "ping-pong tile: 256 or 128 columns");
  constexpr int SLOTF = BM * BKP;
  constexpr unsigned OOB = 0x80000000u;
  extern __shared__ __attribute__((aligned(16))) float smem[];
  auto a_slot = [&](int sl) { return smem + (sl < 2 ? sl : 3) * SLOTF; };
  auto w_slot = [&](int sl) { return smem + (sl == 0 ? 2 : 4) * SLOTF; };
  const int lane = tid & 63;
  const int wave = __builtin_amdgcn_readfirstlane(tid >> 6);
  const int wm = BNW == 256 ? wave >> 2 : wave >> 1, wn = BNW == 256 ? wave & 3 : wave & 1;
  const int group = wave >> 2;
  const int HoWo = g.Ho * g.Wo;
  const int np = TAPI ? (g.Cin / BKP) * __builtin_popcount(tt.mask) : g.Kp / BKP;
  const int k1_pairs = g.A2 ? g.K1 / BKP : 0x7fffffff;
  const int KHKW = g.KH * g.KW;
  const int r_kw = 65536 / g.KW + 1;

  auto set_tap = [&](PpLoader& L) {
    if constexpr (TAPI) {
      const int t = __builtin_ctz(L.a_bits);
      const int kh = (t * r_kw) >> 16, kw = t - kh * g.KW;
#pragma unroll
      for (int it = 0; it < 4; ++it) L.voff[it] = (L.mask[it] >> t) & 1u ? L.row_off[it] : OOB;
      L.seg_soff = (int)((((long)kh * g.Wd + kw) * g.a_pix_stride) * 4);
      return;
    }
#pragma unroll
    for (int it = 0; it < 4; ++it) {
      const int hi = (L.hw0[it] >> 16) + L.is_kh, wi = (int)(short)(L.hw0[it] & 0xffff) + L.is_kw;
      const bool inb = (unsigned)hi < (unsigned)g.H && (unsigned)wi < (unsigned)g.Wd;
      L.voff[it] = inb ? L.row_off[it] : OOB;
    }
    L.seg_soff = (int)((((long)L.is_kh * g.Wd + L.is_kw) * g.a_pix_stride) * 4);
  };
  const int pix_img = TAPI ? tt.ny * tt.nx : HoWo, pix_row = TAPI ? tt.nx : g.Wo;
  const int rows_all = TAPI ? tt.cnt : g.M;
  const float r_howo = 1.0f / (float)pix_img, r_wo = 1.0f / (float)pix_row;
  auto row_pixel = [&](int m0, int rem0, int row, int* dimg_out, int* ho_out, int* wo_out) {
    const bool ok = m0 + row < rows_all;
    const int x = rem0 + (ok ? row : 0);
    int dimg = (int)((float)x * r_howo);
    dimg -= (dimg * pix_img > x);
    dimg += ((dimg + 1) * pix_img <= x);
    const int rem = x - dimg * pix_img;
    int ho = (int)((float)rem * r_wo);
    ho -= (ho * pix_row > rem);
    ho += ((ho + 1) * pix_row <= rem);
    *dimg_out = dimg;
    *wo_out = rem - ho * pix_row + (TAPI ? tt.x0 : 0);
    *ho_out = ho + (TAPI ? tt.y0 : 0);
    return ok;
  };
  auto setup = [&](PpLoader& L, int tm, int tn) {
    const int prow = lane >> 3, pos = lane & 7;
    const int m0 = tm * BM;
    const int img0 = m0 / pix_img;
    const int rem0 = m0 - img0 * pix_img;
    const long bias = ((long)g.pad * g.Wd + g.pad) * g.a_pix_stride;
    L.srd_a = __builtin_amdgcn_make_buffer_rsrc(
        const_cast<float*>(g.A + (long)img0 * g.a_img_stride - bias), 0, 0x7fffffff, 0x00020000);
    L.srd_a2 = __builtin_amdgcn_make_buffer_rsrc(
        const_cast<float*>(g.A2 ? g.A2 + (long)img0 * g.a2_img_stride : g.A), 0, 0x7fffffff,
        0x00020000);
    L.srd_w = __builtin_amdgcn_make_buffer_rsrc(const_cast<float*>(g.W + (long)tn * BNW * g.Kp), 0,
                                                0x7fffffff, 0x00020000);
#pragma unroll
    for (int it = 0; it < 4; ++it) {
      const int row = it * 64 + wave * 8 + prow;
      const int q = pos ^ ((row >> 1) & 7);
      int dimg, ho, wo;
      const bool ok = row_pixel(m0, rem0, row, &dimg, &ho, &wo);
      const int hi0 = ho * g.stride - g.pad, wi0 = wo * g.stride - g.pad;
      L.hw0[it] = (hi0 << 16) | (wi0 & 0xffff);
      if constexpr (TAPI) {
        unsigned m = 0;
        for (int kh = 0, t = 0; kh < g.KH; ++kh)
          for (int kw = 0; kw < g.KW; ++kw, ++t)
            m |= (unsigned)((unsigned)(hi0 + kh) < (unsigned)g.H &&
                            (unsigned)(wi0 + kw) < (unsigned)g.Wd) << t;
        L.mask[it] = m;
      }
      L.row_off[it] = ok ? (unsigned)(((long)dimg * g.a_img_stride +
                                       ((long)hi0 * g.Wd + wi0) * g.a_pix_stride + bias + q * 4) * 4)
                         : OOB;
      L.row_off2[it] = (ok && g.A2)
                           ? (unsigned)(((long)dimg * g.a2_img_stride +
                                         ((long)(ho * g.stride2) * g.W2d + wo * g.stride2) *
                                             g.a2_pix_stride + q * 4) * 4)
                           : OOB;
      L.vb[it] = (row < BNW && tn * BNW + row < g.N) ? (unsigned)(((long)row * g.Kp + q * 4) * 4) : OOB;
    }
    L.ia = L.iw = L.is_kh = L.is_kw = L.is_cin0 = 0;
    L.a_bits = L.w_bits = tt.mask;
    L.w_slice = 0;
    L.cin_limit = g.Cin;
    L.cur_srd = L.srd_a;
    set_tap(L);
  };
  auto issue_a = [&](PpLoader& L, auto slot_tag, bool really) {
    constexpr int SLOT = decltype(slot_tag)::value;
    if (really) {
      int woff = wave * (8 * BKP);
      asm volatile("" : "+s"(woff));
      float* dst = a_slot(SLOT) + woff;
      const int soff = L.seg_soff + L.is_cin0 * 4;
#pragma unroll
      for (int it = 0; it < 4; ++it)
        __builtin_amdgcn_raw_ptr_buffer_load_lds(L.cur_srd, (LDS_AS void*)(dst + it * (64 * BKP)), 16,
                                                 L.voff[it], soff, 0, 0);
    }
    if constexpr (TAPI) {
      if (L.ia + 1 < np) {
        ++L.ia;
        L.a_bits &= L.a_bits - 1;
        if (L.a_bits == 0) { L.a_bits = tt.mask; L.is_cin0 += BKP; }
        set_tap(L);
      }
      return;
    }
    if (L.ia + 1 < np) {
      ++L.ia;
      L.is_cin0 += BKP;
      if (L.ia == k1_pairs) {
        L.cur_srd = L.srd_a2;
#pragma unroll
        for (int it = 0; it < 4; ++it) L.voff[it] = L.row_off2[it];
        L.seg_soff = 0;
        L.is_cin0 = 0;
        L.cin_limit = 0x7fffffff;
      } else if (L.is_cin0 >= L.cin_limit) {
        L.is_cin0 = 0;
        if (++L.is_kw == g.KW) { L.is_kw = 0; ++L.is_kh; }
        set_tap(L);
      }
    }
  };
  auto issue_w = [&](PpLoader& L, auto slot_tag, bool really) {
    constexpr int SLOT = decltype(slot_tag)::value;
    if (really) {
      int woff = wave * (8 * BKP);
// ... 111 lines not shown
    read_frags(sa_tag, sw_tag, I0{});
    issue_w(L, std::integral_constant<int, SLW ^ 1>{}, true);
    asm volatile("s_waitcnt lgkmcnt(0)" ::: "memory");
  };
  auto read_odd = [&](auto sa_tag, auto sw_tag) {
    constexpr int SLA = decltype(sa_tag)::value;
    read_frags(sa_tag, sw_tag, I1{});
    issue_a(L, std::integral_constant<int, (SLA + 2) % 3>{}, true);
    asm volatile("s_waitcnt lgkmcnt(0)" ::: "memory");
  };

  issue_a(L, I0{}, !prefetched);
  issue_w(L, I0{}, !prefetched);
  issue_a(L, I1{}, !prefetched);
  asm volatile("s_waitcnt vmcnt(4)" ::: "memory");
  phase_barrier();
  int left = np;
  if (group == 0) {
    read_even(I0{}, I0{});
    phase_barrier();
    auto pair = [&](auto sa_tag, auto sw_tag) {
      constexpr int SLA = decltype(sa_tag)::value, SLW = decltype(sw_tag)::value;
      multiply();
      phase_barrier();
      read_odd(sa_tag, sw_tag);
      phase_barrier();
      multiply();
      asm volatile("s_waitcnt vmcnt(4)" ::: "memory");
      phase_barrier();
      read_even(std::integral_constant<int, (SLA + 1) % 3>{}, std::integral_constant<int, SLW ^ 1>{});
      phase_barrier();
    };
    for (;;) {
      pair(std::integral_constant<int, 0>{}, I0{});
      if (--left == 0) break;
      pair(std::integral_constant<int, 1>{}, I1{});
      if (--left == 0) break;
      pair(std::integral_constant<int, 2>{}, I0{});
      if (--left == 0) break;
      pair(std::integral_constant<int, 0>{}, I1{});
      if (--left == 0) break;
      pair(std::integral_constant<int, 1>{}, I0{});
      if (--left == 0) break;
      pair(std::integral_constant<int, 2>{}, I1{});
      if (--left == 0) break;
    }
  } else {
    phase_barrier();
    auto pair = [&](auto sa_tag, auto sw_tag) {
      read_even(sa_tag, sw_tag);
      phase_barrier();
      multiply();
      phase_barrier();
      read_odd(sa_tag, sw_tag);
      asm volatile("s_waitcnt vmcnt(4)" ::: "memory");
      phase_barrier();
      multiply();
      phase_barrier();
    };
    for (;;) {
      pair(std::integral_constant<int, 0>{}, I0{});
      if (--left == 0) break;
      pair(std::integral_constant<int, 1>{}, I1{});
      if (--left == 0) break;
      pair(std::integral_constant<int, 2>{}, I0{});
      if (--left == 0) break;
      pair(std::integral_constant<int, 0>{}, I1{});
      if (--left == 0) break;
      pair(std::integral_constant<int, 1>{}, I0{});
      if (--left == 0) break;
      pair(std::integral_constant<int, 2>{}, I1{});
      if (--left == 0) break;
    }
  }
  asm volatile("s_waitcnt vmcnt(0)" ::: "memory");
  __builtin_amdgcn_s_barrier();
  if (has_next) {
    PpLoader N;
    setup(N, ntile_m, ntile_n);
    issue_a(N, I0{}, true);
    issue_w(N, I0{}, true);
    issue_a(N, I1{}, true);
  }
  const GemmArgs ge = reload_gemm_args();
#pragma unroll
  for (int i = 0; i < TM; ++i)
#pragma unroll
    for (int j = 0; j < TN; ++j) acc[i][j] = acc[i][j] * ge.acc_scale;
  if constexpr (TAPI) {
    int* tab = reinterpret_cast<int*>(a_slot(0)) + wave * (TM * 32);
    const int m0 = tile_m * BM;
    const int img0 = m0 / pix_img;
    const int rem0 = m0 - img0 * pix_img;
#pragma unroll
    for (int e = 0; e < TM * 32 / 64; ++e) {
      const int r = e * 64 + lane;
      int dimg, ho, wo;
      const bool ok = row_pixel(m0, rem0, wm * (TM * 32) + r, &dimg, &ho, &wo);
      tab[r] = ok ? ((img0 + dimg) * ge.Ho + ho) * ge.Wo + wo : 0x7fffffff;
    }
    run_epilogue<TM, TN, true, true>(ge, acc, a_slot(2), wave, lane, 0, tile_n * BNW + wn * 64, tab);
  } else {
    run_epilogue<TM, TN, true>(ge, acc, a_slot(2), wave, lane, tile_m * BM + wm * (TM * 32),
                               tile_n * BNW + wn * 64);
  }
}

template <int BNW>
__global__ __launch_bounds__(512, 2) void igemm_split16_pp32n_kernel(GemmArgs g, int tiles_m,
                                                                     int tiles_n) {
  tiles_m = live_tiles_m(g, tiles_m, 256);
  const int T = tiles_m * tiles_n;
  int q = blockIdx.x;
  if (q >= T) return;
  bool prefetched = false;
  for (;;) {
    const int tile = xcd_tile(q, T);
    const int tile_m = tile / tiles_n, tile_n = tile - tile_m * tiles_n;
    const bool has_next = q + (int)gridDim.x < T;
    int ntile_m = tile_m, ntile_n = tile_n;
    if (has_next) {
      const int nt = xcd_tile(q + gridDim.x, T);
      ntile_m = nt / tiles_n;
      ntile_n = nt - ntile_m * tiles_n;
    }
    int tid = threadIdx.x;
    asm volatile("" : "+v"(tid));
    split16_pp32_tile<BNW>(tile_m, tile_n, tid, prefetched, has_next, ntile_m, ntile_n);
    if (!has_next) break;
    asm volatile("s_waitcnt vmcnt(0)" ::: "memory");
    __builtin_amdgcn_s_barrier();
    q += gridDim.x;
    prefetched = true;
  }
}

__global__ __launch_bounds__(512, 2) void igemm_split16_pp32_kernel(GemmArgs g, int tiles_m,
                                                                    int tiles_n) {
  tiles_m = live_tiles_m(g, tiles_m, 256);
  const int T = tiles_m * tiles_n;
  const int q = blockIdx.x;
  if (q >= T) return;
  const int tile = xcd_tile(q, T);
  const int tile_m = tile / tiles_n, tile_n = tile - tile_m * tiles_n;
  int tid = threadIdx.x;
  asm volatile("" : "+v"(tid));
  split16_pp32_tile<256>(tile_m, tile_n, tid, false, false, tile_m, tile_n);
}

template <int BNW>
__global__ __launch_bounds__(512, 2) void igemm_split16_pp32t_kernel(GemmArgs g, int tiles_m,
                                                                     int tiles_n) {
  tiles_m = live_tiles_m(g, tiles_m, 256);
  TapTile tt;
  if (!tap_tile(g, tiles_m, tiles_n, &tt)) return;
  int tid = threadIdx.x;
  asm volatile("" : "+v"(tid));
  split16_pp32_tile<BNW, false, true>(tt.j, tt.tile_n, tid, false, false, tt.j, tt.tile_n, tt);
}

template <int BNW, bool TAPI>
__global__ __launch_bounds__(512, 2) void igemm_f16_pp32_kernel(GemmArgs g, int tiles_m, int tiles_n) {
  tiles_m = live_tiles_m(g, tiles_m, 256);
  if constexpr (TAPI) {
    TapTile tt;
    if (!tap_tile(g, tiles_m, tiles_n, &tt)) return;
    int tid = threadIdx.x;
    asm volatile("" : "+v"(tid));
    split16_pp32_tile<BNW, true, true>(tt.j, tt.tile_n, tid, false, false, tt.j, tt.tile_n, tt);
  } else {
    const int T = tiles_m * tiles_n;
    const int q = blockIdx.x;
    if (q >= T) return;
    const int tile = xcd_tile(q, T);
    const int tile_m = tile / tiles_n, tile_n = tile - tile_m * tiles_n;
    int tid = threadIdx.x;
    asm volatile("" : "+v"(tid));
    split16_pp32_tile<BNW, true, false>(tile_m, tile_n, tid, false, false, tile_m, tile_n);
  }
}

__global__ __launch_bounds__(512, 2) void igemm_split16_pp_kernel(GemmArgs g, int tiles_m,
                                                                  int tiles_n) {
  tiles_m = live_tiles_m(g, tiles_m, 256);
  const int T = tiles_m * tiles_n;
  for (int q = blockIdx.x; q < T; q += gridDim.x) {
    const int tile = xcd_tile(q, T);
    const int tile_m = tile / tiles_n;
    int tid = threadIdx.x;
    asm volatile("" : "+v"(tid));
    split16_pp_tile(tile_m, tile - tile_m * tiles_n, tid);
    __builtin_amdgcn_s_barrier();
  }
}

template <int BM, int BN, int STAGES>
__global__ __launch_bounds__((BM / 64) * (BN / 64) * 64, 2) void igemm_split16_tm2_kernel(
    GemmArgs g, int tiles_m, int tiles_n) {
  tiles_m = live_tiles_m(g, tiles_m, BM);
  if ((int)blockIdx.x >= tiles_m * tiles_n) return;
  const int tile = xcd_tile(blockIdx.x, tiles_m * tiles_n);
  const int tile_m = tile / tiles_n;
  split16_tile<BM, BN, STAGES, 0, 2>(g, tile_m, tile - tile_m * tiles_n);
}


#if MILAN_EXPERIMENTS
template <int BN>
__global__ __launch_bounds__(2 * (BN / 64) * 64, 2) void conv3x3_split16_kernel(
    GemmArgs g, int tiles_m, int tiles_n) {
  constexpr int BM = 256, BK = 16, TM = 4, TN = 2, STAGES = 4, AHEAD = 3;
  constexpr int WAVES_N = BN / 64;
  constexpr int NT = 2 * WAVES_N * 64;
  constexpr int LROWS = NT / 4;
  constexpr int B_ITERS = BN / LROWS;
  constexpr int SROWS = 384;
  constexpr int A_PIECES = SROWS / LROWS;
  static_assert(B_ITERS == 2 && A_PIECES <= 9, "tile configuration");
  extern __shared__ __attribute__((aligned(16))) float smem[];
  float* Bs = smem;
  float* As = smem + STAGES * BN * BK;
  float* Zs = As + 2 * SROWS * BK;
  float* Ds = Zs + 16;

  const int tid = threadIdx.x;
  const int lane = tid & 63;
  const int wave = __builtin_amdgcn_readfirstlane(tid >> 6);
  const int wm = wave / WAVES_N, wn = wave % WAVES_N;
  const int tile = xcd_tile(blockIdx.x, tiles_m * tiles_n);
  const int tile_m = tile / tiles_n, tile_n = tile - tile_m * tiles_n;
  if (tid < 16) Zs[tid] = 0.f;

  const int Wd = g.Wd, H = g.H, Cin = g.Cin;
  const long m0 = (long)tile_m * BM;
  const long total_px = (long)g.M;
  const int halo = Wd + 1;
  const int nchunks = Cin / BK;
  const int nk = nchunks * 9;

  const int lrow = tid >> 2;
  const int lchunk = tid & 3;
// ... 403 lines not shown
  const int pgrid = persist / 8 * 8 * (NT == 256 ? 2 : 1);
  if (persist >= 8 && grid > pgrid) grid = pgrid;
#endif
  hipLaunchKernelGGL(kern, dim3(grid), dim3(NT), lds, s, g, tiles_m, tiles_n);
  MILAN_CHECK_HIP(hipGetLastError());
  return 0;
}

template <int BM, int BN, int STAGES>
static int launch_split16_tm2(const GemmArgs& g, hipStream_t s) {
  const int tiles_m = (g.M + BM - 1) / BM, tiles_n = (g.N + BN - 1) / BN;
  constexpr int NT = (BM / 64) * (BN / 64) * 64;
  size_t lds = size_t(STAGES) * (BM + BN) * 16 * sizeof(float);
  const size_t stage_bytes = size_t(NT / 64) * 32 * 68 * sizeof(float);
  if (lds < stage_bytes) lds = stage_bytes;
  auto kern = igemm_split16_tm2_kernel<BM, BN, STAGES>;
  MILAN_TRY(ensure_lds_attr(reinterpret_cast<const void*>(kern), (int)lds));
  hipLaunchKernelGGL(kern, dim3(tiles_m * tiles_n), dim3(NT), lds, s, g, tiles_m,
                     tiles_n);
  MILAN_CHECK_HIP(hipGetLastError());
  return 0;
}

static bool tap_inner_wanted(const GemmArgs& g) {
  static int on = -1;
  if (on < 0) { const char* e = getenv("MILAN_TAP_INNER"); on = e ? atoi(e) : 1; }
  return on && g.Wt && !g.A2 && g.KH * g.KW > 1 && g.KH * g.KW <= 32 && g.K == g.Kp &&
         g.Cin % 32 == 0;
}

static int tap_classes(GemmArgs& t, int tiles_m, int tiles_n) {
  static int on = -1;
  if (on < 0) { const char* e = getenv("MILAN_TAP_SKIP"); on = e ? atoi(e) : 1; }
  const bool wanted = on && t.tap_ncls >= 0;
  t.tap_ncls = 0;
  const int howo = t.Ho * t.Wo;
  if (!wanted || howo <= 0 || t.M % howo != 0 || (t.m_live && t.m_live_mul % howo != 0))
    return tiles_m * tiles_n;
  struct Run { int o0, n; unsigned set; };
  auto runs = [](int size, int out, int k, int stride, int pad, Run* r) {
    int n = 0;
    for (int o = 0; o < out; ++o) {
      unsigned set = 0;
      for (int i = 0; i < k; ++i)
        if (o * stride - pad + i >= 0 && o * stride - pad + i < size) set |= 1u << i;
      if (n > 0 && r[n - 1].set == set) { ++r[n - 1].n; continue; }
      if (n == MILAN_TAP_CLASSES) return MILAN_TAP_CLASSES + 1;
      r[n++] = Run{o, 1, set};
    }
    return n;
  };
  Run ry[MILAN_TAP_CLASSES], rx[MILAN_TAP_CLASSES];
  const int nry = runs(t.H, t.Ho, t.KH, t.stride, t.pad, ry);
  const int nrx = runs(t.Wd, t.Wo, t.KW, t.stride, t.pad, rx);
  if (nry * nrx > MILAN_TAP_CLASSES) return tiles_m * tiles_n;
  int cls[MILAN_TAP_CLASSES][5], n = 0, min_pix = howo;
  for (int a = 0; a < nry; ++a)
    for (int b = 0; b < nrx; ++b, ++n) {
      unsigned mask = 0;
      for (int kh = 0; kh < t.KH; ++kh)
        for (int kw = 0; kw < t.KW; ++kw)
          if ((ry[a].set >> kh & 1u) && (rx[b].set >> kw & 1u)) mask |= 1u << (kh * t.KW + kw);
      if (mask == 0) return tiles_m * tiles_n;
      const int c[5] = {ry[a].o0, ry[a].n, rx[b].o0, rx[b].n, (int)mask};
      int at = n;
      while (at > 0 && __builtin_popcount((unsigned)cls[at - 1][4]) < __builtin_popcount(mask)) {
        memcpy(cls[at], cls[at - 1], sizeof(c));
        --at;
      }
      memcpy(cls[at], c, sizeof(c));
      if (ry[a].n * rx[b].n < min_pix) min_pix = ry[a].n * rx[b].n;
    }
  if ((256L / min_pix + 2) * t.a_img_stride * 4 + 64 >= 0x7fffffffL) return tiles_m * tiles_n;
  const long imgs = t.M / howo;
  long grid = 0;
  for (int c = 0; c < n; ++c)
    grid += ((imgs * cls[c][1] * cls[c][3] + 255) / 256 * tiles_n + 7) / 8 * 8;
  if (grid >= 0x7fffffffL) return tiles_m * tiles_n;
  t.tap_ncls = n;
  memcpy(t.tap_cls, cls, sizeof(int) * 5 * n);
  return (int)grid;
}

template <int BNW>
static int launch_split16_pp32(const GemmArgs& g, hipStream_t s) {
  const int tiles_m = (g.M + 255) / 256, tiles_n = (g.N + BNW - 1) / BNW;
  const size_t lds = size_t(5) * 256 * 32 * sizeof(float);
  if (tap_inner_wanted(g)) {
    GemmArgs t = g;
    t.W = g.Wt;
    t.tap_inner = 1;
    const int grid = tap_classes(t, tiles_m, tiles_n);
    profile_tag_kernel(BNW == 256 ? MILAN_KERNEL_PP32T_256 : MILAN_KERNEL_PP32_128);
    auto kern = igemm_split16_pp32t_kernel<BNW>;
    MILAN_TRY(ensure_lds_attr(reinterpret_cast<const void*>(kern), (int)lds));
    hipLaunchKernelGGL(kern, dim3(grid), dim3(512), lds, s, t, tiles_m, tiles_n);
    MILAN_CHECK_HIP(hipGetLastError());
    return 0;
  }
  int ncus = 0;
  MILAN_TRY(device_cus8(&ncus));
  int grid = tiles_m * tiles_n;
  static int persist = -1;
  if (persist < 0) { const char* e = getenv("MILAN_PP_PERSIST"); persist = e ? atoi(e) : 0; }
  const bool walk = persist && (persist != 2 || g.K <= 512) && grid > ncus;
  profile_tag_kernel(BNW == 256 ? MILAN_KERNEL_PP32_256 : MILAN_KERNEL_PP32_128);
  if (BNW == 256 && !walk) {
    auto kern = igemm_split16_pp32_kernel;
    MILAN_TRY(ensure_lds_attr(reinterpret_cast<const void*>(kern), (int)lds));
    hipLaunchKernelGGL(kern, dim3(grid), dim3(512), lds, s, g, tiles_m, tiles_n);
  } else {
    auto kern = igemm_split16_pp32n_kernel<BNW>;
    MILAN_TRY(ensure_lds_attr(reinterpret_cast<const void*>(kern), (int)lds));
    if (walk) grid = ncus;
    hipLaunchKernelGGL(kern, dim3(grid), dim3(512), lds, s, g, tiles_m, tiles_n);
  }
  MILAN_CHECK_HIP(hipGetLastError());
  return 0;
}

template <int BNW>
static int launch_f16_pp32(const GemmArgs& g, hipStream_t s) {
  const int tiles_m = (g.M + 255) / 256, tiles_n = (g.N + BNW - 1) / BNW;
  const size_t lds = size_t(5) * 256 * 32 * sizeof(float);
  profile_tag_kernel(MILAN_KERNEL_F16);
  if (tap_inner_wanted(g)) {
    GemmArgs t = g;
    t.W = g.Wt;
    t.tap_inner = 1;
    const int grid = tap_classes(t, tiles_m, tiles_n);
    auto kern = igemm_f16_pp32_kernel<BNW, true>;
    MILAN_TRY(ensure_lds_attr(reinterpret_cast<const void*>(kern), (int)lds));
    hipLaunchKernelGGL(kern, dim3(grid), dim3(512), lds, s, t, tiles_m, tiles_n);
    MILAN_CHECK_HIP(hipGetLastError());
    return 0;
  }
  auto kern = igemm_f16_pp32_kernel<BNW, false>;
  MILAN_TRY(ensure_lds_attr(reinterpret_cast<const void*>(kern), (int)lds));
  hipLaunchKernelGGL(kern, dim3(tiles_m * tiles_n), dim3(512), lds, s, g, tiles_m, tiles_n);
  MILAN_CHECK_HIP(hipGetLastError());
  return 0;
}

static int launch_split16_pp(const GemmArgs& g, hipStream_t s) {
  const int tiles_m = (g.M + 255) / 256, tiles_n = (g.N + 255) / 256;
  const size_t lds = size_t(4) * (256 + 256) * 16 * sizeof(float);
  static_assert(size_t(4) * 512 * 16 * sizeof(float) >= size_t(8) * 32 * 68 * sizeof(float),
                "the epilogue stages through the ring");
  auto kern = igemm_split16_pp_kernel;
  MILAN_TRY(ensure_lds_attr(reinterpret_cast<const void*>(kern), (int)lds));
  hipLaunchKernelGGL(kern, dim3(tiles_m * tiles_n), dim3(512), lds, s, g, tiles_m, tiles_n);
  MILAN_CHECK_HIP(hipGetLastError());
  return 0;
}

static bool pp_eligible(const GemmArgs& g) {
  if (g.Cin % 16 != 0 || g.aniso) return false;
  if (g.A2 && (g.K1 % 16 != 0)) return false;
  const long howo = (long)g.Ho * g.Wo;
  const long imgs = 256 / (howo > 0 ? howo : 1) + 2;
  const long a_span = imgs * g.a_img_stride * 4 + 64;
  const long a2_span = g.A2 ? imgs * g.a2_img_stride * 4 + 64 : 0;
  const long w_span = 256L * g.Kp * 4;
  return a_span < 0x7fffffffL && a2_span < 0x7fffffffL && w_span < 0x7fffffffL;
}

template <int BM, int BN, int STAGES>
static int launch_split16(const GemmArgs& g, hipStream_t s) {
  if constexpr (BM == 256 && BN == 128 && STAGES == 3) {
    static int pp128 = -1;
// ... 14 lines not shown
  }
#if MILAN_EXPERIMENTS
  static int shape = -1;
  if (shape < 0) { const char* e = getenv("MILAN_SCHED"); shape = e ? atoi(e) : 0; }
  if (shape == 1) return launch_split16_impl<BM, BN, STAGES, 1>(g, s);
#endif
#if MILAN_EXPERIMENTS
  if (g.chunk_major) return launch_split16_impl<BM, BN, STAGES, 2>(g, s);
  static int lin = -1;
  if (lin < 0) { const char* e = getenv("MILAN_LINEAR_KERNEL"); lin = e ? atoi(e) : 1; }
  if (!lin) return launch_split16_impl<BM, BN, STAGES, 0>(g, s);
#endif
  if (g.KH == 1 && g.KW == 1 && g.pad == 0 && g.A2 == nullptr) {
    if constexpr (BM == 256 && BN == 256 && STAGES == 5) {
      int cus = 0;
      MILAN_TRY(device_cus8(&cus));
      bool on = true;
#if MILAN_EXPERIMENTS
      static int plin = -1;
      if (plin < 0) { const char* e = getenv("MILAN_PERSIST_LIN"); plin = e ? atoi(e) : 1; }
      on = plin != 0;
#endif
      const int tiles_m = (g.M + BM - 1) / BM, tiles_n = (g.N + BN - 1) / BN;
      if (on && g.Kp / 16 >= STAGES - 1 && tiles_m * tiles_n > cus) {
        const size_t lds = size_t(STAGES) * (BM + BN) * 16 * sizeof(float);
        auto kern = igemm_split16_linp_kernel<STAGES>;
        MILAN_TRY(ensure_lds_attr(reinterpret_cast<const void*>(kern), (int)lds));
        hipLaunchKernelGGL(kern, dim3(cus), dim3(512), lds, s, g, tiles_m, tiles_n);
        MILAN_CHECK_HIP(hipGetLastError());
        return 0;
      }
    }
    return launch_split16_impl<BM, BN, STAGES, 3>(g, s);
  }
  return launch_split16_impl<BM, BN, STAGES, 0>(g, s);
}

static bool aligned16(const void* p) {
  return (reinterpret_cast<uintptr_t>(p) & 15) == 0;
}

#if MILAN_EXPERIMENTS
static int env_tile_hint() {
  static int v = -1;
  if (v < 0) {
    const char* e = getenv("MILAN_TILE_HINT");
    v = e ? atoi(e) : 0;
  }
  return v;
}

static int env_tile_override(int N, int K) {
  static std::vector<int> table;
  static bool parsed = false;
  if (!parsed) {
    parsed = true;
    const char* e = getenv("MILAN_TILE_OVERRIDE");
    while (e && *e) {
      int n = 0, k = 0, h = 0, used = 0;
      if (sscanf(e, "%d:%d:%d%n", &n, &k, &h, &used) == 3) {
        table.push_back(n); table.push_back(k); table.push_back(h);
        e += used;
        if (*e == ',') ++e;
      } else {
        break;
      }
    }
  }
  for (size_t i = 0; i + 2 < table.size(); i += 3)
    if (table[i] == N && table[i + 1] == K) return table[i + 2];
  return 0;
}

static bool conv3x3_enabled() {
  static int v = -1;
  if (v < 0) { const char* e = getenv("MILAN_CONV3X3"); v = e ? atoi(e) != 0 : 0; }
  return v != 0;
}

#else
static int env_tile_hint() { return 0; }
static int env_tile_override(int, int) { return 0; }
#endif

static int launch_gemm_impl(GemmArgs g, hipStream_t s) {
  const bool cin32 = (g.Cin % 32 == 0);
  if (g.status == nullptr) g.status = status_word();
  if (g.tile_hint == 0) g.tile_hint = env_tile_hint();
  if (const int o = env_tile_override(g.N, g.K)) g.tile_hint = o;
  {
    static int dbg = -1;
    if (dbg < 0) { const char* e = getenv("MILAN_ABLATE"); dbg = e ? atoi(e) : 0; }
    g.debug = dbg;
#if MILAN_EXPERIMENTS
    static int stg = -1;
    if (stg < 0) { const char* e = getenv("MILAN_STAGGER"); stg = e ? atoi(e) : 0; }
    static int stg_all = -1;
    if (stg_all < 0) { const char* e = getenv("MILAN_STAGGER_ALL"); stg_all = e ? atoi(e) : 0; }
    g.stagger = (stg_all || (g.out_split && g.N >= 256 && g.KH == 1 && g.H > 1 && (g.aux || g.A2))) ? stg : 0;
#endif
  }
  if (g.epilogue == EPI_LSE) {
    MILAN_REQUIRE(!g.out_split && !g.aux_split && !g.f16 && g.aux == nullptr && g.N % 4 == 0 &&
                      g.ldc == 2 * ((g.N + 63) / 64) && g.C && g.lse_tgt && g.lse_x &&
                      (g.bias == nullptr || aligned16(g.bias)),
                  MILAN_ERR_SHAPE, "gemm: bad log-sum-exp epilogue geometry (N=%d ldc=%d)", g.N,
                  g.ldc);
    g.out_mode = OUT_VEC4;
  } else if (g.epilogue == EPI_LSTM) {
    MILAN_REQUIRE(!g.out_split && !g.aux_split && g.N % 64 == 0 && g.ldc % 8 == 0 &&
                      g.ldaux % 4 == 0 && g.C && g.C2 && g.aux && aligned16(g.C) &&
                      aligned16(g.C2) && aligned16(g.aux) &&
                      (g.Cs == nullptr || aligned16(g.Cs)) &&
                      (g.bias == nullptr || aligned16(g.bias)),
                  MILAN_ERR_SHAPE, "gemm: bad LSTM epilogue geometry (N=%d ldc=%d)",
                  g.N, g.ldc);
    g.out_mode = OUT_VEC4;
  } else if (g.f16) {
    MILAN_REQUIRE(g.a_split && !g.out_split && !g.aux_split && g.N % 8 == 0 && g.ldc % 4 == 0 &&
                      aligned16(g.C) && (g.bias == nullptr || aligned16(g.bias)) &&
                      (g.aux == nullptr || (g.ldaux % 4 == 0 && aligned16(g.aux))) &&
                      (g.epilogue == EPI_BIAS || g.epilogue == EPI_BIAS_RELU ||
                       g.epilogue == EPI_BIAS_RES_RELU) &&
                      g.Cin % 32 == 0 && (!g.A2 || g.K1 % 32 == 0) && g.N >= 128 &&
                      !g.chunk_major && ((long)g.H + g.pad) < 32768 && ((long)g.Wd + g.pad) < 32768,
                  MILAN_ERR_SHAPE, "gemm: unsupported fast-mode (f16) layer N=%d Cin=%d epi=%d",
                  g.N, g.Cin, g.epilogue);
    g.out_mode = OUT_F16;
  } else if (g.out_split || g.aux_split) {
    MILAN_REQUIRE(g.out_split && g.N % 8 == 0 && g.ldc % 8 == 0 && aligned16(g.C) &&
                      (g.bias == nullptr || aligned16(g.bias)) &&
                      (g.aux == nullptr ||
                       ((g.aux_split || g.epilogue == EPI_BIAS_SIGMUL) &&
                        g.ldaux % 8 == 0 && aligned16(g.aux))) &&
                      (g.epilogue == EPI_BIAS || g.epilogue == EPI_BIAS_RELU ||
                       g.epilogue == EPI_BIAS_RES_RELU ||
                       g.epilogue == EPI_BIAS_ADD ||
                       (g.epilogue == EPI_BIAS_SIGMUL && !g.aux_split)),
                  MILAN_ERR_SHAPE,
                  "gemm: unsupported split-format epilogue (N=%d ldc=%d epi=%d)",
                  g.N, g.ldc, g.epilogue);
    g.out_mode = OUT_SPLIT8;
  } else {
    const bool vec_ok = (g.N % 4 == 0) && (g.ldc % 4 == 0) && aligned16(g.C) &&
                        (g.bias == nullptr || aligned16(g.bias)) &&
                        (g.aux == nullptr ||
                         ((g.ldaux % 4 == 0) && aligned16(g.aux)));
    g.out_mode = vec_ok ? OUT_VEC4 : OUT_SCALAR;
  }
  MILAN_REQUIRE(g.A2 == nullptr || (g.a_split && g.N > 64 &&
                                    g.KH == 1 && g.KW == 1 && g.K1 % 16 == 0 &&
                                    (g.tile_hint == 0 || g.tile_hint >= 3)),
                MILAN_ERR_SHAPE, "gemm: two-source A needs the split16 kernels");
  if (g.a_split) {
    if (g.acc_scale == 0.f) g.acc_scale = 1.f;
    if (g.f16) {
      MILAN_REQUIRE(pp_eligible(g), MILAN_ERR_SHAPE, "gemm: fast-mode layer exceeds the 32-bit "
                    "buffer offsets of the ping-pong kernel");
      return g.N % 256 == 0 ? launch_f16_pp32<256>(g, s) : launch_f16_pp32<128>(g, s);
    }
    if (!cin32) {
      MILAN_REQUIRE(g.Cin % 8 == 0 && g.N <= 64 && !g.A2, MILAN_ERR_SHAPE,
                    "gemm: split-f16 operands with Cin %% 32 != 0 need "
                    "Cin %% 8 == 0 and N <= 64 (Cin=%d N=%d)", g.Cin, g.N);
      return launch_cfg<256, 64, 2, false, true>(g, s);
    }
    if (g.N <= 64 && g.tile_hint != 10 && !g.A2 &&
        (g.tile_hint == 6 || (g.tile_hint == 0 && g.KH * g.KW > 1)))
      return launch_split16_tm2<256, 64, 3>(g, s);
    if (g.N <= 64) return launch_cfg<256, 64, 2, true, true>(g, s);
    MILAN_REQUIRE(!g.chunk_major || (MILAN_EXPERIMENTS && g.tile_hint == 0 && !g.A2 && g.Cin % 16 == 0),
                  MILAN_ERR_SHAPE, "gemm: chunk-major k order: experiments build, split16 kernels");
#if MILAN_EXPERIMENTS
    if (g.W3 && g.KH == 3 && g.KW == 3 && g.stride == 1 && g.pad == 1 && !g.A2 &&
        g.Cin % 16 == 0 && g.a_pix_stride == g.Cin && g.Ho == g.H && g.Wo == g.Wd &&
        g.a_img_stride == (long)g.H * g.Wd * g.Cin && g.Wd + 1 <= 64 &&
        (g.tile_hint == 8 || (g.tile_hint == 0 && conv3x3_enabled()))) {
      if (g.N % 256 == 0) return launch_conv3x3<256>(g, s);
      if (g.N % 128 == 0) return launch_conv3x3<128>(g, s);
    }
#endif
#if MILAN_EXPERIMENTS
    if (g.tile_hint == 3) return launch_split16<256, 256, 4>(g, s);
    if (g.tile_hint == 7) return launch_split16<256, 256, 5>(g, s);
    if (g.tile_hint == 4) return launch_split16<256, 128, 3>(g, s);
    if (g.tile_hint == 5) return launch_split16<128, 256, 3>(g, s);
    if (g.tile_hint == 1) return launch_cfg<256, 128, 3, true, true>(g, s);
    if (g.tile_hint == 2) return launch_cfg<128, 128, 2, true, true>(g, s);
#endif
    if (g.N % 256 == 0) return launch_split16<256, 256, 5>(g, s);
    {
      const int pad256 = (g.N + 255) / 256 * 256 - g.N;
      const int pad128 = (g.N + 127) / 128 * 128 - g.N;
      if (g.N > 2048 && pad256 <= pad128)
        return launch_split16<256, 256, 5>(g, s);
    }
    return launch_split16<256, 128, 3>(g, s);
  }
  if (g.N <= 64) {
    return cin32 ? launch_cfg<256, 64, 2, true, false>(g, s)
                 : launch_cfg<256, 64, 2, false, false>(g, s);
  }
#if MILAN_EXPERIMENTS
  if (cin32 && g.tile_hint == 1)
    return launch_cfg<256, 128, 3, true, false>(g, s);
#endif
  return cin32 ? launch_cfg<128, 128, 2, true, false>(g, s)
               : launch_cfg<128, 128, 2, false, false>(g, s);
}

int launch_gemm(const GemmArgs& g, hipStream_t s) {
  MILAN_REQUIRE(g.M > 0 && g.N > 0 && g.K > 0, MILAN_ERR_SHAPE,
                "gemm: empty problem M=%d N=%d K=%d", g.M, g.N, g.K);
  MILAN_REQUIRE(g.Cin % 4 == 0 && g.a_pix_stride % 4 == 0 &&
                    g.a_img_stride % 4 == 0 && g.Kp % 32 == 0 && aligned16(g.A) &&
                    aligned16(g.W),
                MILAN_ERR_SHAPE,
                "gemm: Cin=%d / strides must be multiples of 4 floats and "
                "operands 16-byte aligned", g.Cin);
  if (!g_prof.on) return launch_gemm_impl(g, s);
  ProfRec* e = prof_next();
  MILAN_REQUIRE(e != nullptr, MILAN_ERR_STATE, "profiler: cannot create events");
  e->stage = g_prof.stage;
  e->gemm = true;
  e->kernel = g.a_split ? MILAN_KERNEL_SPLIT_OTHER : MILAN_KERNEL_F32;
  e->flops = 2.0 * (double)g.M * (double)g.N * (double)(g.flop_k > 0 ? g.flop_k : g.K);
  e->bytes = gemm_algorithmic_bytes(g);
  g_prof.open = e;
  MILAN_CHECK_HIP(hipEventRecord(e->a, s));
  const int r = launch_gemm_impl(g, s);
  g_prof.open = nullptr;
  MILAN_CHECK_HIP(hipEventRecord(e->b, s));
  return r;
}

}
```

### neuron-descriptions_amd/milan_amd/hip.py

```python
import ctypes
import os
import pathlib
import weakref
from typing import Dict, Optional, Sequence, Tuple

import torch

LIB_PATH = pathlib.Path(os.environ.get('MILAN_LIB') or
                       pathlib.Path(__file__).resolve().parent / 'lib' / 'libmilan_hip.so')
EXP_LIB_PATH = pathlib.Path(__file__).resolve().parent / 'lib' / 'libmilan_hip_exp.so'

GREEDY, FORCED, BEAM, RERANK = 0, 1, 2, 3
PRECISION_F32, PRECISION_SPLIT_F16, PRECISION_F16 = 0, 1, 2
PRECISIONS = {'f32': PRECISION_F32, 'split_f16': PRECISION_SPLIT_F16, 'f16': PRECISION_F16}
FUSE_CHAIN, FUSE_CHAIN_WIDE, FUSE_STEM, FUSE_CONV3, FUSE_SKIP_EMPTY, FUSE_BNECK, FUSE_SPARSE_TAIL = 1, 2, 4, 8, 16, 32, 64
SKETCH_COMPACT, SKETCH_INSERT, SKETCH_MOVE, SKETCH_HALVE = 0, 1, 2, 3
STATUS_SATURATED, STATUS_NONFINITE_INPUT = 1, 2
KERNEL_FAMILIES = ('other', 'pp32_256', 'pp32_128', 'split_other', 'f32', 'chain',
                   'chain_wide', 'stem', 'conv3', 'f16', 'pp32t_256', 'bneck')


class SketchOp(ctypes.Structure):
    _fields_ = [('kind', ctypes.c_int32), ('src', ctypes.c_int32),
                ('dst', ctypes.c_int32), ('offset', ctypes.c_int32),
                ('extremes', ctypes.c_int32), ('reserved', ctypes.c_int32),
                ('n', ctypes.c_int64), ('position', ctypes.c_int64),
                ('capacity', ctypes.c_int64)]


DRAW_BIT = ctypes.CFUNCTYPE(ctypes.c_int, ctypes.c_void_p)
_CONV_PRECISIONS = dict(f32=0, split_f16=1, split_f16_strip=3, split_f16_tap_major=4,
                        split_f16_tap_linear=5)
DTYPE_U8, DTYPE_F32 = 0, 1

ERR_ARG, ERR_SHAPE, ERR_STATE, ERR_WORKSPACE, ERR_NO_LM = -1, -2, -3, -4, -5


class HipUnavailableError(RuntimeError):
    """libmilan_hip.so or a HIP device is missing."""


class Dims(ctypes.Structure):
    _fields_ = [
        ('trunk_width', ctypes.c_int32),
        ('trunk_blocks', ctypes.c_int32 * 4),
        ('feature_size', ctypes.c_int32),
        ('hidden_size', ctypes.c_int32),
        ('embedding_size', ctypes.c_int32),
        ('attention_size', ctypes.c_int32),
        ('vocab_size', ctypes.c_int32),
        ('start_index', ctypes.c_int32),
        ('stop_index', ctypes.c_int32),
        ('pad_index', ctypes.c_int32),
        ('has_lm', ctypes.c_int32),
        ('lm_hidden_size', ctypes.c_int32),
        ('lm_embedding_size', ctypes.c_int32),
        ('lm_layers', ctypes.c_int32),
        ('trunk_kind', ctypes.c_int32),
    ]


class ClipDims(ctypes.Structure):
    _fields_ = [(name, ctypes.c_int32) for name in (
        'resolution', 'patch', 'vision_width', 'vision_layers', 'vision_heads',
        'embed_dim', 'context_length', 'vocab_size', 'text_width',
        'text_layers', 'text_heads')]


class BertDims(ctypes.Structure):
    _fields_ = [(name, ctypes.c_int32) for name in (
        'vocab_size', 'width', 'layers', 'heads', 'intermediate',
        'max_positions', 'type_vocab', 'position_offset')] + [('eps', ctypes.c_float)]


BERT_MAX_TOKENS = 64

ABI_VERSION = 11

TRUNK_BOTTLENECK, TRUNK_BASIC, TRUNK_ALEXNET, TRUNK_NONE = 0, 1, 2, 3
_FEATURE_MULT = {TRUNK_BOTTLENECK: 61, TRUNK_BASIC: 16, TRUNK_ALEXNET: 18}


_P = ctypes.c_void_p
_I = ctypes.c_int
_F = ctypes.c_float
_SZ = ctypes.c_size_t
_I64 = ctypes.c_int64

SIGNATURES = {
    'milan_abi_version': (_I, []),
    'milan_last_error': (ctypes.c_char_p, []),
    'milan_create': (_I, [ctypes.POINTER(_P), _I,
                          ctypes.POINTER(Dims)]),
    'milan_destroy': (None, [_P]),
    'milan_set_weight':
        (_I, [_P, ctypes.c_char_p, _P,
              ctypes.POINTER(ctypes.c_int64), _I]),
    'milan_finalize_weights': (_I, [_P, _P]),
# ... 202 lines not shown
        torch.cuda.synchronize()
        torch.cuda.empty_cache()


def _kfd_gpuids(pid) -> set:
    ids = set()
    try:
        base = f'/sys/class/kfd/kfd/proc/{pid}/queues'
        for q in os.listdir(base):
            try:
                with open(f'{base}/{q}/gpuid') as f:
                    ids.add(f.read().strip())
            except OSError:
                pass
    except OSError:
        pass
    return ids


def other_compute_processes() -> list:
    mine = _kfd_gpuids(os.getpid())
    if not mine:
        return []
    try:
        pids = [int(p) for p in os.listdir('/sys/class/kfd/kfd/proc') if p.isdigit()]
    except OSError:
        return []
    return sorted(p for p in pids if p != os.getpid() and _kfd_gpuids(p) & mine)


_SHARED_WARNED = False


def warn_if_gpu_is_shared() -> None:
    global _SHARED_WARNED
    others = other_compute_processes()
    if others and not _SHARED_WARNED:
        _SHARED_WARNED = True
        import warnings
        warnings.warn(
            f'milan_amd: {len(others)} other process(es) have compute queues on a GPU '
            f'this process uses (pids {others[:4]}{"..." if len(others) > 4 else ""}): '
            'kernels of two processes can become co-resident on a CU, which is '
            'unsupported on this platform (see INTEGRATION.md, "One process per GPU")',
            RuntimeWarning, stacklevel=3)


class Context:

    def __init__(self, dims: Dims, state_dict: Dict[str, torch.Tensor],
                 device: torch.device, finalize: bool = True):
        self.lib = load_library()
        self.device = require_device(device)
        self.dims = dims
        self._h = _P()
        with torch.cuda.device(self.device):
            _check(
                self.lib.milan_create(ctypes.byref(self._h), self.device.index,
                                      ctypes.byref(dims)))
            keep = []
            for name, tensor in state_dict.items():
                if not tensor.dtype.is_floating_point:
                    continue
                t = _dev(tensor.detach(), self.device, torch.float32)
                keep.append(t)
                shape = (ctypes.c_int64 * max(1, t.dim()))(*t.shape)
                _check(
                    self.lib.milan_set_weight(self._h, name.encode(),
                                              t.data_ptr(), shape, t.dim()))
            if finalize:
                _check(
                    self.lib.milan_finalize_weights(self._h,
                                                    _stream(self.device)))
            del keep
        self._ws: Optional[torch.Tensor] = None
        self.on_saturation = os.environ.get('MILAN_ON_SATURATION', 'raise')
        self.saturation_fallbacks = 0
        _LIVE_CONTEXTS.add(self)
        warn_if_gpu_is_shared()
        if os.environ.get('MILAN_CHAIN'):
            bits = int(os.environ['MILAN_CHAIN'])
            self.set_fusion(chain=bool(bits & 1), wide=bool(bits & 2), stem=bool(bits & 4),
                            conv3=bool(bits & 8), skip_empty=bool(bits & 16),
                            bneck=bool(bits & 32), sparse_tail=bool(bits & 64))
        if os.environ.get('MILAN_SHARE_IMAGES'):
            self.set_image_sharing(bool(int(os.environ['MILAN_SHARE_IMAGES'])))
        default = os.environ.get('MILAN_PRECISION')
        if default == 'auto':
            self.set_precision('split_f16')
            self.on_saturation = 'f32'
        elif default:
            self.set_precision(default)

    def enable_graphs(self, enable: bool = True) -> None:
        _check(self.lib.milan_set_graph_capture(self._h, int(enable)))
        self._graphs = bool(enable)
        if enable and getattr(self, '_gstream', None) is None:
            self._gstream = torch.cuda.Stream(device=self.device)
            self._pool = {}

    def graph_stats(self):
        cap, rep = ctypes.c_longlong(), ctypes.c_longlong()
        _check(self.lib.milan_graph_stats(self._h, ctypes.byref(cap),
                                          ctypes.byref(rep)))
        return cap.value, rep.value

    def _pooled(self, key, make):
        buf = self._pool.get(key)
        if buf is None:
            self._pool[key] = buf = make()
        return buf

    def set_precision(self, precision) -> None:
        if isinstance(precision, str):
            if precision not in PRECISIONS:
                raise ValueError(f'unknown precision: {precision}')
            precision = PRECISIONS[precision]
        _check(self.lib.milan_set_precision(self._h, int(precision)))

    def set_fusion(self, chain: bool = True, wide: Optional[bool] = None,
                   stem: bool = True, conv3: bool = True, skip_empty: bool = True,
                   bneck: bool = True, sparse_tail: bool = True) -> None:
        wide = chain if wide is None else wide
        _check(self.lib.milan_set_fusion(
            self._h, (FUSE_CHAIN if chain else 0) | (FUSE_CHAIN_WIDE if wide else 0) |
            (FUSE_STEM if stem else 0) | (FUSE_CONV3 if conv3 else 0) |
            (FUSE_SKIP_EMPTY if skip_empty else 0) | (FUSE_BNECK if bneck else 0) |
            (FUSE_SPARSE_TAIL if sparse_tail else 0)))

    def set_image_sharing(self, enable: bool = True) -> None:
        _check(self.lib.milan_set_image_sharing(self._h, int(bool(enable))))

    @property
    def image_sharing(self) -> bool:
        return bool(self.lib.milan_get_image_sharing(self._h))

    def image_sharing_stats(self, clear: bool = False) -> Tuple[int, int]:
        slots, trunk = ctypes.c_longlong(), ctypes.c_longlong()
        with torch.cuda.device(self.device):
            _check(self.lib.milan_image_sharing_stats(self._h, ctypes.byref(slots),
                                                      ctypes.byref(trunk), int(clear),
                                                      _stream(self.device)))
        return int(slots.value), int(trunk.value)

    @property
    def precision(self) -> str:
        code = self.lib.milan_get_precision(self._h)
        return {v: k for k, v in PRECISIONS.items()}[code]

    def status(self, clear: bool = True) -> int:
        flags = ctypes.c_uint32(0)
        with torch.cuda.device(self.device):
            _check(self.lib.milan_status(self._h, ctypes.byref(flags), int(clear),
                                         _stream(self.device)))
        return int(flags.value)

    @property
    def act_scale_log2(self) -> int:
        return int(self.lib.milan_get_act_scale_log2(self._h))

    def set_act_scale_log2(self, k: int) -> None:
        with torch.cuda.device(self.device):
            _check(self.lib.milan_set_act_scale_log2(self._h, int(k),
                                                     _stream(self.device)))

    def encoder_absmax(self, images: torch.Tensor) -> float:
        m, ch, h, w = images.shape
        if ch != 3:
            raise ValueError(f'images must have 3 channels, got {ch}')
        idt = DTYPE_U8 if images.dtype == torch.uint8 else DTYPE_F32
        images = _dev(images, self.device, None if idt == DTYPE_U8 else torch.float32)
        ws = self.workspace(m or 1, 1, max(h, w), 1, 1)
        out = _F(0.0)
        with torch.cuda.device(self.device):
            _check(self.lib.milan_encoder_absmax(self._h, images.data_ptr(), idt, m, h, w,
                                                 ctypes.byref(out), ws.data_ptr(),
                                                 ws.numel(), _stream(self.device)))
        return float(out.value)

    def calibrate(self, images: torch.Tensor, headroom: float = 8.0) -> int:
        import math
        amax = self.encoder_absmax(images)
        if not math.isfinite(amax):
            raise FloatingPointError('calibration sample produced non-finite activations')
        k = 10 if amax <= 0 else int(math.floor(math.log2(65504.0 / (amax * headroom))))
        k = max(0, min(10, k))
        self.set_act_scale_log2(k)
        return k

    def _guarded(self, what: str, run, check: bool = True):
        out = run()
        if not check or self.on_saturation == 'ignore':
            return out
        flags = self.status(clear=True)
        if flags & STATUS_NONFINITE_INPUT:
            import warnings
            warnings.warn(f'milan_amd: {what}: an input image holds NaN / Inf pixels; its '
                          'features are NaN (as in the reference)', RuntimeWarning,
                          stacklevel=3)
        if flags & STATUS_SATURATED:
            limit = 65504.0 / 2 ** self.act_scale_log2
            msg = (f'milan_amd: {what}: a split-f16 activation exceeded {limit:g} '
                   f'(65504 / 2^{self.act_scale_log2}) and was clamped; the exact-fp32 '
                   "mode (precision='f32'), Decoder.precision = 'auto' or a smaller "
                   'activation scale (Context.calibrate) avoid it')
            if self.on_saturation != 'f32' or self.precision == 'f32':
                raise FloatingPointError(msg)
            import warnings
            warnings.warn(msg + ' -- rerunning this call in f32', RuntimeWarning,
                          stacklevel=3)
            self.saturation_fallbacks += 1
# ... 987 lines not shown
```

Baseline: 1380.

## Run sparse-tail convolutions as row-list GEMMs and extend sparsity into layer3

Adds a row-list mode to the split-f16 pp32 GEMM kernel, so each launch computes only the output pixels named in a compacted per-image list instead of full dense tiles. The mode is enabled by default under a new TAIL_LISTS fusion flag. New kernels derive layer3 pixel sets by back-projecting the layer4 live pixels through the 3x3 and downsample receptive fields. This lets the first layer4 block and the last layer3 block also skip unneeded rows. The cost is extra set, scan and fill kernels, more workspace, indirect row gathers in the epilogue, and a more complex dispatch that must stay in sync with row_list_supported.

```diff
diff --git a/include/milan_hip.h b/include/milan_hip.h
--- a/include/milan_hip.h
+++ b/include/milan_hip.h
@@ -124,7 +124,8 @@
        MILAN_FUSE_CONV3 = 8,
        MILAN_FUSE_SKIP_EMPTY = 16,
        MILAN_FUSE_BNECK = 32,
-       MILAN_FUSE_SPARSE_TAIL = 64 };
+       MILAN_FUSE_SPARSE_TAIL = 64,
+       MILAN_FUSE_TAIL_LISTS = 128 };
 int milan_set_fusion(milan_ctx* ctx, int flags);
 int milan_set_precision(milan_ctx* ctx, int precision);
 int milan_get_precision(const milan_ctx* ctx);
diff --git a/neuron-descriptions_amd/csrc/api.hip b/neuron-descriptions_amd/csrc/api.hip
--- a/neuron-descriptions_amd/csrc/api.hip
+++ b/neuron-descriptions_amd/csrc/api.hip
@@ -484,8 +484,11 @@
 int milan_set_fusion(milan_ctx* c, int flags) {
   MILAN_REQUIRE(c, MILAN_ERR_ARG, "null ctx");
   MILAN_REQUIRE((flags & ~(MILAN_FUSE_CHAIN | MILAN_FUSE_CHAIN_WIDE | MILAN_FUSE_STEM | MILAN_FUSE_CONV3 |
-                           MILAN_FUSE_SKIP_EMPTY | MILAN_FUSE_BNECK | MILAN_FUSE_SPARSE_TAIL)) == 0, MILAN_ERR_ARG,
+                           MILAN_FUSE_SKIP_EMPTY | MILAN_FUSE_BNECK | MILAN_FUSE_SPARSE_TAIL |
+                           MILAN_FUSE_TAIL_LISTS)) == 0, MILAN_ERR_ARG,
                 "unknown fusion flags %d", flags);
+  MILAN_REQUIRE(!(flags & MILAN_FUSE_TAIL_LISTS) || (flags & MILAN_FUSE_SPARSE_TAIL), MILAN_ERR_ARG,
+                "MILAN_FUSE_TAIL_LISTS needs MILAN_FUSE_SPARSE_TAIL (flags %d)", flags);
   c->fusion = flags;
   return 0;
 }
diff --git a/neuron-descriptions_amd/csrc/common.h b/neuron-descriptions_amd/csrc/common.h
--- a/neuron-descriptions_amd/csrc/common.h
+++ b/neuron-descriptions_amd/csrc/common.h
@@ -88,6 +88,7 @@
   long lse_tgt_stride;
   float* lse_x;
   const int* m_live;
+  const int* row_list;
   int m_live_mul;
   int tap_ncls;
   int tap_cls[MILAN_TAP_CLASSES][5];
@@ -97,6 +98,7 @@
 enum OutMode : int { OUT_SCALAR = 0, OUT_VEC4 = 1, OUT_SPLIT8 = 2, OUT_F16 = 3 };
 
 int launch_gemm(const GemmArgs& g, hipStream_t s);
+bool row_list_supported(const GemmArgs& g);
 void set_status_word(unsigned* word);
 unsigned* status_word();
 void profile_tag_kernel(int family);
@@ -382,7 +384,8 @@
   int precision = 0;
   int trunk_f16 = 0;
   int fusion = MILAN_FUSE_CHAIN | MILAN_FUSE_CHAIN_WIDE | MILAN_FUSE_STEM | MILAN_FUSE_CONV3 |
-               MILAN_FUSE_SKIP_EMPTY | MILAN_FUSE_BNECK | MILAN_FUSE_SPARSE_TAIL;
+               MILAN_FUSE_SKIP_EMPTY | MILAN_FUSE_BNECK | MILAN_FUSE_SPARSE_TAIL |
+               MILAN_FUSE_TAIL_LISTS;
   int graph_capture = 0;
   struct GraphEntry { std::vector<char> key; hipGraphExec_t exec = nullptr; int seen = 0; };
   std::vector<GraphEntry> graphs;
diff --git a/neuron-descriptions_amd/csrc/encoder.hip b/neuron-descriptions_amd/csrc/encoder.hip
--- a/neuron-descriptions_amd/csrc/encoder.hip
+++ b/neuron-descriptions_amd/csrc/encoder.hip
@@ -875,11 +875,11 @@
 
 __global__ __launch_bounds__(64) void tail_union_kernel(
     const int* __restrict__ list_idx, const int* __restrict__ list_n, Levels lv,
-    const int* __restrict__ class_of, int P, unsigned char* __restrict__ s0) {
+    const int* __restrict__ class_of, int P, unsigned char* __restrict__ s0, int level) {
   const int i = blockIdx.x, c = class_of[i];
   if (c < 0) return;
-  const long base = (long)i * lv.per_image + lv.off[4];
-  const int cnt = list_n[i * 5 + 4];
+  const long base = (long)i * lv.per_image + lv.off[level];
+  const int cnt = list_n[i * 5 + level];
   for (int e = threadIdx.x; e < cnt; e += 64) s0[(long)c * P + list_idx[base + e]] = 1;
 }
 
@@ -887,7 +887,7 @@
     const int* __restrict__ list_idx, const int* __restrict__ list_n, Levels lv,
     const int* __restrict__ order, const int* __restrict__ live, int n,
     int* __restrict__ loc, int* __restrict__ cnt,
-    const unsigned char* __restrict__ s0 = nullptr) {
+    const unsigned char* __restrict__ s0, int dummy) {
   __shared__ unsigned char s[3][kTailMaxP];
   const int j = blockIdx.x, lane = threadIdx.x;
   const int h = lv.h[4], w = lv.w[4], P = h * w;
@@ -906,6 +906,12 @@
     for (int i = lane; i < c; i += 64) s[0][list_idx[base + i]] = 1;
   }
   __syncthreads();
+  if (dummy) {
+    int any = 0;
+    for (int p = lane; p < P; p += 64) any |= s[0][p];
+    if (__ballot(any != 0) == 0ull && lane == 0) s[0][0] = 1;
+    __syncthreads();
+  }
   for (int k = 1; k < 3; ++k) {
     for (int p = lane; p < P; p += 64) {
       const int y = p / w, x = p - y * w;
@@ -930,6 +936,59 @@
       count += __popcll(m);
     }
     if (lane == 0) cnt[k * n + j] = count;
+  }
+}
+
+constexpr int kTailMaxP3 = 4096;
+__global__ __launch_bounds__(64) void tail_sets3_kernel(
+    const int* __restrict__ loc, const int* __restrict__ cnt, int k0,
+    const int* __restrict__ list_idx, const int* __restrict__ list_n, Levels lv,
+    const int* __restrict__ order, const int* __restrict__ live, int n, int kh, int kw,
+    int stride, int pad, int ds_stride, const unsigned char* __restrict__ s3,
+    int* __restrict__ loc3, int* __restrict__ cnt3) {
+  __shared__ unsigned char s[2][kTailMaxP3];
+  const int j = blockIdx.x, lane = threadIdx.x;
+  const int w4 = lv.w[4], P4 = lv.h[4] * w4;
+  const int h3 = lv.h[3], w3 = lv.w[3], P3 = h3 * w3;
+  if (live != nullptr && j >= *live) {
+    if (lane < 2) cnt3[lane * n + j] = 0;
+    return;
+  }
+  for (int p = lane; p < P3; p += 64) {
+    s[0][p] = 0;
+    s[1][p] = s3 != nullptr ? s3[(long)j * P3 + p] : 0;
+  }
+  __syncthreads();
+  if (s3 == nullptr) {
+    const int img = order ? order[j] : j;
+    const long base = (long)img * lv.per_image + lv.off[3];
+    const int c = list_n[img * 5 + 3];
+    for (int i = lane; i < c; i += 64) s[1][list_idx[base + i]] = 1;
+  }
+  const int c0 = cnt[k0 * n + j];
+  const int* l0 = loc + ((long)k0 * n + j) * P4;
+  for (int i = lane; i < c0; i += 64) {
+    const int p = l0[i], y = p / w4, x = p - y * w4;
+    for (int a = 0; a < kh; ++a)
+      for (int b = 0; b < kw; ++b) {
+        const int yy = y * stride - pad + a, xx = x * stride - pad + b;
+        if (yy >= 0 && yy < h3 && xx >= 0 && xx < w3) { s[0][yy * w3 + xx] = 1; s[1][yy * w3 + xx] = 1; }
+      }
+    const int yd = y * ds_stride, xd = x * ds_stride;
+    if (yd < h3 && xd < w3) s[1][yd * w3 + xd] = 1;
+  }
+  __syncthreads();
+  for (int k = 0; k < 2; ++k) {
+    int count = 0;
+    int* out = loc3 + ((long)k * n + j) * P3;
+    for (int p0 = 0; p0 < P3; p0 += 64) {
+      const int p = p0 + lane;
+      const bool nz = p < P3 && s[k][p];
+      const unsigned long long m = __ballot(nz);
+      if (nz) out[count + __popcll(m & ((1ull << lane) - 1ull))] = p;
+      count += __popcll(m);
+    }
+    if (lane == 0) cnt3[k * n + j] = count;
   }
 }
 
@@ -1011,6 +1070,8 @@
   void* sh_hash;
   int *sh_rep, *sh_flag, *class_of;
   unsigned char* tail_s0;
+  int *tail_loc3, *tail_cnt3, *tail_off3, *tail_rows3, *tail_U3;
+  unsigned char* tail_s3;
 };
 
 static int conv_out(int h, int k, int s, int p) { return (h + 2 * p - k) / s + 1; }
@@ -1067,6 +1128,13 @@
     pl->sh_flag = a.get<int>((size_t)n);
     pl->class_of = a.get<int>((size_t)n);
     pl->tail_s0 = a.get<unsigned char>(((size_t)n * P4 + 3) & ~(size_t)3);
+    const size_t P3 = (size_t)lv.h[3] * lv.w[3];
+    pl->tail_loc3 = a.get<int>(2 * (size_t)n * P3);
+    pl->tail_rows3 = a.get<int>(2 * (size_t)n * P3);
+    pl->tail_cnt3 = a.get<int>(2 * (size_t)n);
+    pl->tail_off3 = a.get<int>(2 * (size_t)n);
+    pl->tail_U3 = a.get<int>(4);
+    pl->tail_s3 = a.get<unsigned char>(((size_t)n * P3 + 3) & ~(size_t)3);
   }
   return 0;
 }
@@ -1460,16 +1528,17 @@
     const size_t need = (size_t)P4 * ((size_t)2 * lb.c1.cin + lb.c3.cout + (size_t)11 * lb.c1.cout);
     tail = need <= (size_t)pl.h1 * pl.w1 * wd;
   }
+  const bool lists = tail && (c->fusion & MILAN_FUSE_TAIL_LISTS);
   if (tail) {
     const unsigned char* s0 = nullptr;
     if (class_of != nullptr) {
       MILAN_TRY(launch_zero_fill(pl.tail_s0, ((size_t)n * P4 + 3) & ~(size_t)3, s));
       hipLaunchKernelGGL(tail_union_kernel, dim3(n), dim3(64), 0, s, pl.list_idx, pl.list_n, pl.lv,
-                         class_of, P4, pl.tail_s0);
+                         class_of, P4, pl.tail_s0, 4);
       s0 = pl.tail_s0;
     }
     hipLaunchKernelGGL(tail_sets_kernel, dim3(n), dim3(64), 0, s, pl.list_idx, pl.list_n, pl.lv,
-                       order, live, n, pl.tail_loc, pl.tail_cnt, s0);
+                       order, live, n, pl.tail_loc, pl.tail_cnt, s0, lists ? 1 : 0);
     hipLaunchKernelGGL(tail_scan_kernel, dim3(3), dim3(256), 0, s, pl.tail_cnt, n, pl.tail_off,
                        pl.tail_U);
     hipLaunchKernelGGL(tail_fill_kernel, dim3(n, 3), dim3(64), 0, s, pl.tail_loc, pl.tail_cnt,
@@ -1526,6 +1595,113 @@
     return 0;
   };
 
+  auto on_list = [&](GemmArgs g, const int* rows, const int* U) {
+    g.row_list = rows; g.m_live = U; g.m_live_mul = 1;
+    return g;
+  };
+  auto list_ok = [&](const GemmArgs& g) { return row_list_supported(on_list(g, pl.tail_rows, pl.tail_U)); };
+  auto tail_block_args = [&](const Bottleneck& b, const float* X, float* Y, float* T1, int hh,
+                             int ww, GemmArgs* g1, GemmArgs* g2, GemmArgs* g3) {
+    int h1, w1, h2, w2, h3, w3;
+    *g1 = conv_args(b.c1, X, n, hh, ww, T1, EPI_BIAS_RELU, nullptr, c->zero, &h1, &w1, true);
+    *g2 = conv_args(b.c2, T1, n, h1, w1, pl.t2, EPI_BIAS_RELU, nullptr, c->zero, &h2, &w2, true);
+    *g3 = conv_args(b.c3, pl.t2, n, h2, w2, Y, EPI_BIAS_RES_RELU, X, c->zero, &h3, &w3, true);
+  };
+  auto tail_block_lists_ok = [&](const Bottleneck& b, int hh, int ww) {
+    GemmArgs g1, g2, g3;
+    tail_block_args(b, pl.x0, pl.x1, pl.t1, hh, ww, &g1, &g2, &g3);
+    return lists && list_ok(g1) && list_ok(g2) && list_ok(g3);
+  };
+  auto tail_block_lists = [&](const Bottleneck& b, const float* X, float* Y, float* T1, int hh,
+                              int ww, int kM, int kO) -> int {
+    GemmArgs g1, g2, g3;
+    tail_block_args(b, X, Y, T1, hh, ww, &g1, &g2, &g3);
+    const int* rowsM = pl.tail_rows + (long)kM * n * P4;
+    const int* rowsO = pl.tail_rows + (long)kO * n * P4;
+    MILAN_TRY(launch_gemm(on_list(g1, rowsM, pl.tail_U + kM), s));
+    MILAN_TRY(launch_gemm(on_list(g2, rowsO, pl.tail_U + kO), s));
+    MILAN_TRY(launch_gemm(on_list(g3, rowsO, pl.tail_U + kO), s));
+    return 0;
+  };
+  auto two_source_args = [&](const Bottleneck& b, const float* xin, float* yo, int hh, int ww,
+                             int h2, int w2, int* h3, int* w3) {
+    GemmArgs g3 = conv_args(b.c3d, pl.t2, n, h2, w2, yo, EPI_BIAS_RELU,
+                            nullptr, c->zero, h3, w3, true);
+    g3.Cin = b.c3.cin;
+    g3.a_pix_stride = b.c3.cin;
+    g3.a_img_stride = (long)h2 * w2 * b.c3.cin;
+    g3.A2 = xin; g3.K1 = b.c3.K; g3.H2 = hh; g3.W2d = ww;
+    g3.stride2 = b.down.stride;
+    g3.a2_pix_stride = b.down.cin;
+    g3.a2_img_stride = (long)hh * ww * b.down.cin;
+    g3.flop_k = b.c3.K + b.down.K;
+    return g3;
+  };
+  const int h3l = pl.lv.h[3], w3l = pl.lv.w[3], P3 = h3l * w3l;
+  int k0 = -1;
+  bool lists_l3 = false;
+  bool lists_down = lists;
+#if MILAN_EXPERIMENTS
+  if (getenv("MILAN_TAPS_INNER") && atoi(getenv("MILAN_TAPS_INNER"))) lists_down = false;
+#endif
+  if (lists_down && c->blocks[3].size() >= 2 && c->blocks[3].size() <= 3 && P3 <= kTailMaxP3) {
+    const std::vector<Bottleneck>& b4 = c->blocks[3];
+    const Bottleneck& f = b4[0];
+    bool ok = true;
+    for (size_t bi = 1; bi < b4.size(); ++bi) ok = ok && tail_block_ok(b4[bi]);
+    ok = ok && !f.basic && f.has_down && f.c3d.ws && f.c3d.cout > 64 && f.c1.kh == 1 && f.c1.kw == 1 &&
+         f.c1.stride == 1 && f.c1.pad == 0 && f.c3.kh == 1 && f.c3.kw == 1 && f.c3.stride == 1 &&
+         f.c3.pad == 0 && f.down.kh == 1 && f.down.kw == 1 && f.down.pad == 0 && f.c2.wst &&
+         f.c1.bias_s && f.c2.bias_s && f.c3d.bias_s &&
+         conv_out(h3l, f.c2.kh, f.c2.stride, f.c2.pad) == pl.lv.h[4] &&
+         conv_out(w3l, f.c2.kw, f.c2.stride, f.c2.pad) == pl.lv.w[4] &&
+         conv_out(h3l, 1, f.down.stride, 0) == pl.lv.h[4] &&
+         conv_out(w3l, 1, f.down.stride, 0) == pl.lv.w[4] &&
+         !(f.down.stride == 1 && (c->fusion & (f.c3.cin >= 256 ? MILAN_FUSE_CHAIN_WIDE : MILAN_FUSE_CHAIN)));
+    if (ok) {
+      int h1, w1, h2, w2, h3, w3;
+      GemmArgs g1 = conv_args(f.c1, pl.x0, n, h3l, w3l, pl.t1, EPI_BIAS_RELU, nullptr, c->zero, &h1, &w1, true);
+      GemmArgs g2 = conv_args(f.c2, pl.t1, n, h1, w1, pl.t2, EPI_BIAS_RELU, nullptr, c->zero, &h2, &w2, true);
+      GemmArgs g3 = two_source_args(f, pl.x0, pl.x1, h3l, w3l, h2, w2, &h3, &w3);
+      ok = list_ok(g1) && list_ok(g2) && list_ok(g3);
+    }
+    if (ok) k0 = (int)b4.size() - 1;
+    const std::vector<Bottleneck>& b3 = c->blocks[2];
+    if (ok && b3.size() >= 2) {
+      const Bottleneck& l = b3.back();
+      bool ok3 = !l.basic && !l.has_down && l.c2.wst && l.c2.bias_s && l.c3.bias_s && l.c2.stride == 1 &&
+                 l.c3.kh == 1 && l.c3.kw == 1 && l.c3.stride == 1 && l.c3.pad == 0 &&
+                 conv_out(h3l, l.c2.kh, 1, l.c2.pad) == h3l && conv_out(w3l, l.c2.kw, 1, l.c2.pad) == w3l;
+      if (ok3) {
+        int h2, w2, h3, w3;
+        GemmArgs g2 = conv_args(l.c2, pl.t1, n, h3l, w3l, pl.t2, EPI_BIAS_RELU, nullptr, c->zero, &h2, &w2, true);
+        GemmArgs g3 = conv_args(l.c3, pl.t2, n, h2, w2, pl.x1, EPI_BIAS_RES_RELU, pl.x0, c->zero, &h3, &w3, true);
+        ok3 = list_ok(g2) && list_ok(g3);
+      }
+      lists_l3 = ok3;
+    }
+  }
+  if (k0 >= 0) {
+    const Bottleneck& f = c->blocks[3][0];
+    const unsigned char* s3 = nullptr;
+    if (class_of != nullptr) {
+      MILAN_TRY(launch_zero_fill(pl.tail_s3, ((size_t)n * P3 + 3) & ~(size_t)3, s));
+      hipLaunchKernelGGL(tail_union_kernel, dim3(n), dim3(64), 0, s, pl.list_idx, pl.list_n, pl.lv,
+                         class_of, P3, pl.tail_s3, 3);
+      s3 = pl.tail_s3;
+    }
+    hipLaunchKernelGGL(tail_sets3_kernel, dim3(n), dim3(64), 0, s, pl.tail_loc, pl.tail_cnt, k0,
+                       pl.list_idx, pl.list_n, pl.lv, order, live, n, f.c2.kh, f.c2.kw, f.c2.stride,
+                       f.c2.pad, f.down.stride, s3, pl.tail_loc3, pl.tail_cnt3);
+    hipLaunchKernelGGL(tail_scan_kernel, dim3(2), dim3(256), 0, s, pl.tail_cnt3, n, pl.tail_off3,
+                       pl.tail_U3);
+    hipLaunchKernelGGL(tail_fill_kernel, dim3(n, 2), dim3(64), 0, s, pl.tail_loc3, pl.tail_cnt3,
+                       pl.tail_off3, n, P3, pl.tail_rows3);
+    MILAN_CHECK_HIP(hipGetLastError());
+  }
+  const int* rowsV = pl.tail_rows3;
+  const int* rowsW = pl.tail_rows3 + (long)n * P3;
+
   float *x = pl.x0, *y = pl.x1;
   int h = pl.hp, w = pl.wp, col = wd;
   bool t1_ready = false;
@@ -1572,7 +1748,8 @@
           (bi + 1 == blocks.size() || tail_block_ok(blocks.back())) &&
           h == pl.lv.h[4] && w == pl.lv.w[4]) {
         const int kO = bi + 1 == blocks.size() ? 0 : 1;
-        MILAN_TRY(tail_block(b, x, y, t1buf, h, w, kO + 1, kO));
+        if (tail_block_lists_ok(b, h, w)) MILAN_TRY(tail_block_lists(b, x, y, t1buf, h, w, kO + 1, kO));
+        else MILAN_TRY(tail_block(b, x, y, t1buf, h, w, kO + 1, kO));
         float* tmp = x; x = y; y = tmp;
         continue;
       }
@@ -1645,6 +1822,26 @@
           b.c1.kw == 1 && b.c1.stride == 1 && b.c1.cin == 64 && b.c1.cout == 64 &&
           b.c1.K == b.c1.Kp && h1 == h && w1 == w &&
           chain_conv_c1_supported(chain_P, b.down.cin, chain_NR, h1, w1);
+      if (k0 >= 0 && li == 3 && bi == 0 && !chain_plain && !chain_ds && h == h3l && w == w3l) {
+        const int* rows0 = pl.tail_rows + (long)k0 * n * P4;
+        if (c1_pending) MILAN_TRY(launch_gemm(on_list(g1, rowsV, pl.tail_U3), s));
+        MILAN_TRY(launch_gemm(on_list(g2, rows0, pl.tail_U + k0), s));
+        GemmArgs g3 = two_source_args(b, x, y, h, w, h2, w2, &h3, &w3);
+        MILAN_TRY(launch_gemm(on_list(g3, rows0, pl.tail_U + k0), s));
+        float* tmp = x; x = y; y = tmp;
+        h = h3; w = w3;
+        continue;
+      }
+      if (lists_l3 && k0 >= 0 && li == 2 && last_of_stage && !chain_plain && !chain_ds &&
+          h == h3l && w == w3l) {
+        if (c1_pending) MILAN_TRY(gemm_t(g1));
+        MILAN_TRY(launch_gemm(on_list(g2, rowsW, pl.tail_U3 + 1), s));
+        GemmArgs g3 = conv_args(b.c3, pl.t2, n, h2, w2, y, EPI_BIAS_RES_RELU, x, c->zero, &h3, &w3, split);
+        MILAN_TRY(launch_gemm(on_list(g3, rowsW, pl.tail_U3 + 1), s));
+        float* tmp = x; x = y; y = tmp;
+        h = h3; w = w3;
+        continue;
+      }
       if (c1_pending && !c1_front) MILAN_TRY(gemm_t(g1));
       if (conv_front) {
       } else if (split && (c->fusion & MILAN_FUSE_CONV3) && b.c2.K == b.c2.Kp &&
@@ -1689,16 +1886,7 @@
       }
       if (b.has_down && split && b.c3d.ws && b.c3d.cout > 64) {
         int h3, w3;
-        GemmArgs g3 = conv_args(b.c3d, pl.t2, n, h2, w2, y, EPI_BIAS_RELU,
-                                nullptr, c->zero, &h3, &w3, true);
-        g3.Cin = b.c3.cin;
-        g3.a_pix_stride = b.c3.cin;
-        g3.a_img_stride = (long)h2 * w2 * b.c3.cin;
-        g3.A2 = x; g3.K1 = b.c3.K; g3.H2 = h; g3.W2d = w;
-        g3.stride2 = b.down.stride;
-        g3.a2_pix_stride = b.down.cin;
-        g3.a2_img_stride = (long)h * w * b.down.cin;
-        g3.flop_k = b.c3.K + b.down.K;
+        GemmArgs g3 = two_source_args(b, x, y, h, w, h2, w2, &h3, &w3);
         MILAN_TRY(gemm_t(g3));
         float* tmp = x; x = y; y = tmp;
         h = h3; w = w3;
diff --git a/neuron-descriptions_amd/csrc/gemm.hip b/neuron-descriptions_amd/csrc/gemm.hip
--- a/neuron-descriptions_amd/csrc/gemm.hip
+++ b/neuron-descriptions_amd/csrc/gemm.hip
@@ -1223,6 +1223,7 @@
   }
 }
 
+template <bool DENSE_M = false>
 __device__ __forceinline__ GemmArgs reload_gemm_args() {
   typedef const int __attribute__((address_space(4)))* KArgWords;
   KArgWords kw = (KArgWords)__builtin_amdgcn_kernarg_segment_ptr();
@@ -1232,7 +1233,8 @@
 #pragma unroll
   for (unsigned i = 0; i < sizeof(GemmArgs) / 4; ++i) words[i] = kw[i];
   __builtin_memcpy(&g, words, sizeof(GemmArgs));
-  g.M = live_rows(g.m_live, g.m_live_mul, g.M);
+  if constexpr (!DENSE_M)
+    g.M = live_rows(g.m_live, g.m_live_mul, g.M);
   return g;
 }
 
@@ -1502,7 +1504,7 @@
   return true;
 }
 
-template <int BNW, bool F16 = false, bool TAPI = false>
+template <int BNW, bool F16 = false, bool TAPI = false, bool LIST = false>
 __device__ __forceinline__ void split16_pp32_tile(int tile_m, int tile_n, int tid, bool prefetched,
                                                   bool has_next, int ntile_m, int ntile_n,
                                                   TapTile tt = TapTile{}) {
@@ -1544,9 +1546,14 @@
   const int pix_img = TAPI ? tt.ny * tt.nx : HoWo, pix_row = TAPI ? tt.nx : g.Wo;
   const int rows_all = TAPI ? tt.cnt : g.M;
   const float r_howo = 1.0f / (float)pix_img, r_wo = 1.0f / (float)pix_row;
+  auto list_slot0 = [&](int m0) {
+    return __builtin_amdgcn_readfirstlane(g.row_list[m0]) / pix_img;
+  };
   auto row_pixel = [&](int m0, int rem0, int row, int* dimg_out, int* ho_out, int* wo_out) {
     const bool ok = m0 + row < rows_all;
-    const int x = rem0 + (ok ? row : 0);
+    int x;
+    if constexpr (LIST) x = g.row_list[m0 + (ok ? row : 0)] - rem0;
+    else x = rem0 + (ok ? row : 0);
     int dimg = (int)((float)x * r_howo);
     dimg -= (dimg * pix_img > x);
     dimg += ((dimg + 1) * pix_img <= x);
@@ -1562,8 +1569,8 @@
   auto setup = [&](PpLoader& L, int tm, int tn) {
     const int prow = lane >> 3, pos = lane & 7;
     const int m0 = tm * BM;
-    const int img0 = m0 / pix_img;
-    const int rem0 = m0 - img0 * pix_img;
+    const int img0 = LIST ? list_slot0(m0) : m0 / pix_img;
+    const int rem0 = LIST ? img0 * pix_img : m0 - img0 * pix_img;
     const long bias = ((long)g.pad * g.Wd + g.pad) * g.a_pix_stride;
     L.srd_a = __builtin_amdgcn_make_buffer_rsrc(
         const_cast<float*>(g.A + (long)img0 * g.a_img_stride - bias), 0, 0x7fffffff, 0x00020000);
@@ -1841,12 +1848,22 @@
     issue_w(N, I0{}, true);
     issue_a(N, I1{}, true);
   }
-  const GemmArgs ge = reload_gemm_args();
+  const GemmArgs ge = reload_gemm_args<LIST>();
 #pragma unroll
   for (int i = 0; i < TM; ++i)
 #pragma unroll
     for (int j = 0; j < TN; ++j) acc[i][j] = acc[i][j] * ge.acc_scale;
-  if constexpr (TAPI) {
+  if constexpr (LIST) {
+    int* tab = reinterpret_cast<int*>(a_slot(0)) + wave * (TM * 32);
+    const int m0 = tile_m * BM;
+#pragma unroll
+    for (int e = 0; e < TM * 32 / 64; ++e) {
+      const int r = e * 64 + lane;
+      const int m = m0 + wm * (TM * 32) + r;
+      tab[r] = m < rows_all ? ge.row_list[m] : 0x7fffffff;
+    }
+    run_epilogue<TM, TN, true, true>(ge, acc, a_slot(2), wave, lane, 0, tile_n * BNW + wn * 64, tab);
+  } else if constexpr (TAPI) {
     int* tab = reinterpret_cast<int*>(a_slot(0)) + wave * (TM * 32);
     const int m0 = tile_m * BM;
     const int img0 = m0 / pix_img;
@@ -1916,6 +1933,26 @@
   int tid = threadIdx.x;
   asm volatile("" : "+v"(tid));
   split16_pp32_tile<BNW, false, true>(tt.j, tt.tile_n, tid, false, false, tt.j, tt.tile_n, tt);
+}
+
+template <bool TAPI>
+__global__ __launch_bounds__(512, 2) void igemm_split16_pp32l_kernel(GemmArgs g, int tiles_m,
+                                                                     int tiles_n) {
+  tiles_m = live_tiles_m(g, tiles_m, 256);
+  const int T = tiles_m * tiles_n;
+  const int q = blockIdx.x;
+  if (q >= T) return;
+  const int tile = xcd_tile(q, T);
+  const int tile_m = tile / tiles_n, tile_n = tile - tile_m * tiles_n;
+  TapTile tt{};
+  if constexpr (TAPI) {
+    tt.ny = g.Ho; tt.nx = g.Wo;
+    tt.mask = 0xffffffffu >> (32 - g.KH * g.KW);
+    tt.cnt = g.M;
+  }
+  int tid = threadIdx.x;
+  asm volatile("" : "+v"(tid));
+  split16_pp32_tile<256, false, TAPI, true>(tile_m, tile_n, tid, false, false, tile_m, tile_n, tt);
 }
 
 template <int BNW, bool TAPI>
@@ -2485,10 +2522,26 @@
   return (int)grid;
 }
 
+static thread_local bool t_row_list_taken = false;
+
 template <int BNW>
 static int launch_split16_pp32(const GemmArgs& g, hipStream_t s) {
   const int tiles_m = (g.M + 255) / 256, tiles_n = (g.N + BNW - 1) / BNW;
   const size_t lds = size_t(5) * 256 * 32 * sizeof(float);
+  if (g.row_list != nullptr) {
+    if (BNW != 256) return MILAN_ERR_SHAPE;
+    t_row_list_taken = true;
+    GemmArgs t = g;
+    const bool tapi = tap_inner_wanted(g);
+    if (tapi) { t.W = g.Wt; t.tap_inner = 1; }
+    t.tap_ncls = 0;
+    profile_tag_kernel(tapi ? MILAN_KERNEL_PP32T_256 : MILAN_KERNEL_PP32_256);
+    auto kern = tapi ? igemm_split16_pp32l_kernel<true> : igemm_split16_pp32l_kernel<false>;
+    MILAN_TRY(ensure_lds_attr(reinterpret_cast<const void*>(kern), (int)lds));
+    hipLaunchKernelGGL(kern, dim3(tiles_m * tiles_n), dim3(512), lds, s, t, tiles_m, tiles_n);
+    MILAN_CHECK_HIP(hipGetLastError());
+    return 0;
+  }
   if (tap_inner_wanted(g)) {
     GemmArgs t = g;
     t.W = g.Wt;
@@ -2669,6 +2722,28 @@
 static int env_tile_hint() { return 0; }
 static int env_tile_override(int, int) { return 0; }
 #endif
+
+bool row_list_supported(const GemmArgs& g) {
+  static int pp = -1;
+  if (pp < 0) { const char* e = getenv("MILAN_PP"); pp = e ? atoi(e) : 1; }
+  const long howo = (long)g.Ho * g.Wo;
+  if (g.row_list == nullptr || g.m_live == nullptr || g.m_live_mul != 1) return false;
+  if (!g.a_split || g.f16 || g.chunk_major || g.aniso || g.tile_hint != 0 || env_tile_hint() != 0 ||
+      env_tile_override(g.N, g.K) != 0 || pp != 1)
+    return false;
+#if MILAN_EXPERIMENTS
+  if (conv3x3_enabled() || (getenv("MILAN_SCHED") && atoi(getenv("MILAN_SCHED")))) return false;
+#endif
+  if (g.epilogue == EPI_LSE || g.epilogue == EPI_LSTM || !g.out_split) return false;
+  if (g.N % 256 != 0 || g.Cin % 32 != 0 || g.K != g.Kp || !pp_eligible(g)) return false;
+  if (g.A2 && (g.K1 % 32 != 0 || g.KH != 1 || g.KW != 1)) return false;
+  if (g.KH * g.KW > 1 && !tap_inner_wanted(g)) return false;
+  if ((long)g.H + g.pad >= 32768 || (long)g.Wd + g.pad >= 32768) return false;
+  if (howo <= 0 || g.M % howo != 0 || 257 * howo >= (1L << 24)) return false;
+  if (258 * g.a_img_stride * 4 + 64 >= 0x7fffffffL) return false;
+  if (g.A2 && 258 * g.a2_img_stride * 4 + 64 >= 0x7fffffffL) return false;
+  return true;
+}
 
 static int launch_gemm_impl(GemmArgs g, hipStream_t s) {
   const bool cin32 = (g.Cin % 32 == 0);
@@ -2796,15 +2871,30 @@
                : launch_cfg<128, 128, 2, false, false>(g, s);
 }
 
+static int launch_gemm_checked(const GemmArgs& g, hipStream_t s);
 int launch_gemm(const GemmArgs& g, hipStream_t s) {
   MILAN_REQUIRE(g.M > 0 && g.N > 0 && g.K > 0, MILAN_ERR_SHAPE,
                 "gemm: empty problem M=%d N=%d K=%d", g.M, g.N, g.K);
+  MILAN_REQUIRE(g.row_list == nullptr || row_list_supported(g), MILAN_ERR_SHAPE,
+                "gemm: no row-list form of this launch (N=%d Cin=%d %dx%d)", g.N, g.Cin, g.KH, g.KW);
   MILAN_REQUIRE(g.Cin % 4 == 0 && g.a_pix_stride % 4 == 0 &&
                     g.a_img_stride % 4 == 0 && g.Kp % 32 == 0 && aligned16(g.A) &&
                     aligned16(g.W),
                 MILAN_ERR_SHAPE,
                 "gemm: Cin=%d / strides must be multiples of 4 floats and "
                 "operands 16-byte aligned", g.Cin);
+  if (g.row_list != nullptr) {
+    t_row_list_taken = false;
+    const int r = launch_gemm_checked(g, s);
+    MILAN_REQUIRE(r != 0 || t_row_list_taken, MILAN_ERR_STATE,
+                  "gemm: a row-list launch was dispatched to a kernel without a list form "
+                  "(row_list_supported() no longer matches the dispatch)");
+    return r;
+  }
+  return launch_gemm_checked(g, s);
+}
+
+static int launch_gemm_checked(const GemmArgs& g, hipStream_t s) {
   if (!g_prof.on) return launch_gemm_impl(g, s);
   ProfRec* e = prof_next();
   MILAN_REQUIRE(e != nullptr, MILAN_ERR_STATE, "profiler: cannot create events");
diff --git a/neuron-descriptions_amd/milan_amd/hip.py b/neuron-descriptions_amd/milan_amd/hip.py
--- a/neuron-descriptions_amd/milan_amd/hip.py
+++ b/neuron-descriptions_amd/milan_amd/hip.py
@@ -14,6 +14,7 @@
 PRECISION_F32, PRECISION_SPLIT_F16, PRECISION_F16 = 0, 1, 2
 PRECISIONS = {'f32': PRECISION_F32, 'split_f16': PRECISION_SPLIT_F16, 'f16': PRECISION_F16}
 FUSE_CHAIN, FUSE_CHAIN_WIDE, FUSE_STEM, FUSE_CONV3, FUSE_SKIP_EMPTY, FUSE_BNECK, FUSE_SPARSE_TAIL = 1, 2, 4, 8, 16, 32, 64
+FUSE_TAIL_LISTS = 128
 SKETCH_COMPACT, SKETCH_INSERT, SKETCH_MOVE, SKETCH_HALVE = 0, 1, 2, 3
 STATUS_SATURATED, STATUS_NONFINITE_INPUT = 1, 2
 KERNEL_FAMILIES = ('other', 'pp32_256', 'pp32_128', 'split_other', 'f32', 'chain',
@@ -382,7 +383,8 @@
             bits = int(os.environ['MILAN_CHAIN'])
             self.set_fusion(chain=bool(bits & 1), wide=bool(bits & 2), stem=bool(bits & 4),
                             conv3=bool(bits & 8), skip_empty=bool(bits & 16),
-                            bneck=bool(bits & 32), sparse_tail=bool(bits & 64))
+                            bneck=bool(bits & 32), sparse_tail=bool(bits & 64),
+                            tail_lists=bool(bits & 128))
         if os.environ.get('MILAN_SHARE_IMAGES'):
             self.set_image_sharing(bool(int(os.environ['MILAN_SHARE_IMAGES'])))
         default = os.environ.get('MILAN_PRECISION')
@@ -420,13 +422,16 @@
 
     def set_fusion(self, chain: bool = True, wide: Optional[bool] = None,
                    stem: bool = True, conv3: bool = True, skip_empty: bool = True,
-                   bneck: bool = True, sparse_tail: bool = True) -> None:
+                   bneck: bool = True, sparse_tail: bool = True,
+                   tail_lists: Optional[bool] = None) -> None:
+        tail_lists = sparse_tail if tail_lists is None else tail_lists
         wide = chain if wide is None else wide
         _check(self.lib.milan_set_fusion(
             self._h, (FUSE_CHAIN if chain else 0) | (FUSE_CHAIN_WIDE if wide else 0) |
             (FUSE_STEM if stem else 0) | (FUSE_CONV3 if conv3 else 0) |
             (FUSE_SKIP_EMPTY if skip_empty else 0) | (FUSE_BNECK if bneck else 0) |
-            (FUSE_SPARSE_TAIL if sparse_tail else 0)))
+            (FUSE_SPARSE_TAIL if sparse_tail else 0) |
+            (FUSE_TAIL_LISTS if tail_lists else 0)))
 
     def set_image_sharing(self, enable: bool = True) -> None:
         _check(self.lib.milan_set_image_sharing(self._h, int(bool(enable))))
```

New measurement: 1418, median of 6. 2.8% higher.
